# bjo5029/causal-vae

Hardware: AMD Instinct MI355X
Metric: training samples/sec on 128^3 vessel volumes (3D CausalVAE train step) (higher is better)
Workload: dtype bf16; 1 GPU; 3D vessel CausalVAE train step, 128^3 bf16 volumes (z-scored N(0,1)), batch 4/GPU, Adam lr 0.0001, ELBO = MSE-sum + 2000*MSE-sum(m) + KLD; global_batch=4, per_gpu_batch=4, parallelism=dp1, params=15346957

## Files before the change

### causal_vae_amd/_lib.py

```python
import ctypes as C
import os

import torch

_HERE = os.path.dirname(os.path.abspath(__file__))
LIB_PATH = os.environ.get("CVAE_HIP_LIB") or os.path.join(_HERE, "libcvae_hip.so")

F32, BF16, FP8 = 0, 1, 2
ACT_NONE, ACT_RELU, ACT_SIGMOID, ACT_LEAKY02, ACT_LEAKY001 = 0, 1, 2, 3, 4
_ACT = {None: ACT_NONE, "none": ACT_NONE, "relu": ACT_RELU, "sigmoid": ACT_SIGMOID, "leaky02": ACT_LEAKY02, "leaky001": ACT_LEAKY001}


class CvaeError(RuntimeError):
    pass


if not os.path.exists(LIB_PATH):
    raise ImportError(
        f"{LIB_PATH} is missing: build it with `python -c 'import __graft_entry__ as g; g.build()'` "
        "(or `make -C causal_vae_amd/csrc`).  causal_vae_amd has no CPU / eager fallback.")
lib = C.CDLL(LIB_PATH)

_p, _i64, _i, _f, _sz, _u64 = C.c_void_p, C.c_int64, C.c_int, C.c_float, C.c_size_t, C.c_uint64

SIGNATURES = {
    "cvae_version": [],
    "cvae_strerror": [_i],
    "cvae_ncs_to_nsc": [_p, _p, _i64, _i64, _i64, _i, _i, _p],
    "cvae_nsc_to_ncs": [_p, _p, _i64, _i64, _i64, _i, _i, _p],
    "cvae_cast": [_p, _p, _i64, _i, _i, _p],
    "cvae_copy_panels": [_p, _p, _p, _i, _p, _i64, _i64, _i64, _i, _p],
    "cvae_onehot_panel": [_p, _p, _i64, _i64, _i64, _i64, _p],
    "cvae_conv_pack_weight": [_p, _p, _i64, _i64, _i, _i, _i, _p],
    "cvae_conv_pack_weight_pairs": [_p, _p, _p, _p, _p, _p, _p, _p, _p, _i, _i, _i, _p],
    "cvae_conv_data_workspace_bytes": [_i64] * 9 + [_i, _i],
    "cvae_conv_down": [_p] * 7 + [_i64] * 9 + [_i, _i, _i, _p, _sz, _i, _p],
    "cvae_conv_up": [_p] * 7 + [_i64] * 9 + [_i, _i, _i, _p, _sz, _i, _i, _i64, _p],
    "cvae_conv_down_bwd_data": [_p] * 4 + [_i64] * 7 + [_i, _i, _i, _p, _sz, _i, _i, _p],
    "cvae_quantize_fp8": [_p, _i, _p, _i64, _f, _p, _p, _p],
    "cvae_conv_pack_weight_fp8": [_p, _p, _i64, _i64, _i, _i, _f, _p],
    "cvae_conv_up_c1_fp8in": [_p, _p, _p, _p, _f, _i64, _i64, _i64, _i64, _i64, _i, _i, _p],
    "cvae_absmax": [_p, _i, _i64, _p, _p],
    "cvae_conv_pack_weights_fp8": [_p, _p, _p, _p, _p, _p, _p, _i, _i, _p],
    "cvae_conv_fp8": [_i, _p, _p, _p, _p, _i, _p, _p, _f, _f, _p] + [_i64] * 9 + [_i, _i, _p, _sz, _i, _p, _p],
    "cvae_fp8_scale_update": [_p, _p, _p, _i, _f, _p, _p, _p, _i, _p, _p, _p],
    "cvae_conv_down_image_f8": [_p, _i, _p, _p, _p, _p, _p, _p, _p] + [_i64] * 8 + [_i, _i, _p],
    "cvae_conv_image_supported": [_p, _i64, _i, _i],
    "cvae_conv_down_image": [_p, _i, _p, _p, _p, _p] + [_i64] * 8 + [_i, _i, _i, _p],
    "cvae_conv_wgrad_image": [_p, _p, _i, _p, _p, _p, _sz] + [_i64] * 8 + [_i, _i, _p],
    "cvae_conv_wgrad_workspace_bytes": [_i64, _i64, _i],
    "cvae_conv_wgrad": [_p, _p, _p, _p, _i, _p, _sz] + [_i64] * 9 + [_i, _i, _p],
    "cvae_conv_wgrad_multi": [_i, _p, _p, _p, _p, _p, _p, _p, _p, _i, _i, _p],
    "cvae_channel_sum_workspace_bytes": [_i64, _i64, _i],
    "cvae_channel_sum": [_p, _p, _i64, _i64, _i, _p, _sz, _p],
    "cvae_act_fwd": [_p, _p, _i64, _i, _i, _p],
    "cvae_act_bwd": [_p, _p, _p, _i64, _i, _i, _p],
    "cvae_adaptive_avgpool_fwd": [_p, _p] + [_i64] * 9 + [_i, _p],
    "cvae_adaptive_avgpool_bwd": [_p, _p, _p] + [_i64] * 9 + [_i, _p],
    "cvae_upsample_linear_fwd": [_p, _p] + [_i64] * 8 + [_i, _p],
    "cvae_upsample_linear_bwd": [_p, _p] + [_i64] * 8 + [_i, _p],
    "cvae_linear_workspace_bytes": [_i64, _i64, _i64, _i],
    "cvae_linear_fwd": [_p, _p, _p, _p, _i64, _i64, _i64, _i64, _i64, _i, _i, _p, _sz, _p],
    "cvae_linear_bwd_data": [_p, _p, _p, _i64, _i64, _i64, _i64, _i64, _p, _i, _p, _i64, _i, _i, _p, _sz, _p],
    "cvae_linear_bwd_weight": [_p, _p, _p, _p, _i64, _i64, _i64, _i64, _i64, _p, _i, _i, _p, _sz, _p],
    "cvae_small_dense_supported": [_i64, _i64, _i64],
    "cvae_small_dense_workspace_bytes": [_i64, _i64, _i64],
    "cvae_small_dense_fwd": [_p, _p, _p, _p, _i64, _i64, _i64, _i64, _i64, _i, _p],
    "cvae_small_dense_bwd_data": [_p, _p, _p, _p, _i, _p, _i, _i64, _i64, _i64, _i64, _i64, _i64, _i64, _p],
    "cvae_small_dense_bwd_weight": [_p, _p, _p, _p, _p, _i, _i64, _i64, _i64, _i64, _i64, _i64, _p, _sz, _p],
    "cvae_bn1d_train_fwd": [_p] * 8 + [_i64, _i64, _f, _f, _p],
    "cvae_bn1d_train_bwd": [_p] * 8 + [_i64, _i64, _p],
    "cvae_bn1d_eval_fwd": [_p] * 6 + [_i64, _i64, _f, _p],
    "cvae_bn1d_stats": [_p, _p, _f, _p, _i64, _i64, _p],
    "cvae_bn1d_apply_stats": [_p] * 5 + [_f] + [_p] * 5 + [_i64, _i64, _f, _f, _p],
    "cvae_bn1d_bwd_sums": [_p] * 5 + [_i64, _i64, _p],
    "cvae_bn1d_bwd_apply": [_p] * 6 + [_f, _p, _i64, _i64, _p],
    "cvae_philox_normal": [_p, _i64, _u64, _u64, _u64, _p, _p],
    "cvae_philox_normal_advance": [_p, _i64, _u64, _u64, _u64, _p, _p],
    "cvae_reduce_workspace_bytes": [],
    "cvae_reparam_kld_fwd": [_p, _p, _p, _p, _p, _i64, _p, _sz, _p],
    "cvae_reparam_kld_bwd": [_p, _p, _f] + [_p] * 5 + [_i64, _p],
    "cvae_latent_head_fwd": [_p, _p, _p, _p, _p, _p, _i64, _i64, _p],
    "cvae_latent_head_bwd": [_p, _p, _p, _p, _p, _p, _p, _i64, _i64, _p],
    "cvae_sse_fwd": [_p, _p, _p, _i64, _p, _sz, _p],
    "cvae_sse_bwd": [_p, _p, _p, _f, _p, _i64, _p],
    "cvae_combine3": [_p, _f, _f, _p],
    "cvae_bce_fwd": [_p, _p, _p, _i64, _p, _sz, _p],
    "cvae_bce_bwd": [_p, _p, _p, _p, _i64, _p],
    "cvae_sum_fwd": [_p, _p, _i64, _p, _sz, _p],
    "cvae_wmse_sparsity_fwd": [_p, _p, _p, _p, _i64, _i64, _p, _sz, _p],
    "cvae_wmse_sparsity_bwd": [_p] * 6 + [_i64, _i64, _p],
    "cvae_gauss_nll_fwd": [_p, _p, _p, _p, _i64, _p, _sz, _p],
    "cvae_gauss_nll_bwd": [_p] * 6 + [_i64, _p],
    "cvae_softmax_ce_fwd": [_p, _p, _p, _i64, _i64, _p, _sz, _p],
    "cvae_softmax_ce_bwd": [_p, _p, _p, _p, _i64, _i64, _p],
    "cvae_uniform_kl_fwd": [_p, _p, _i64, _i64, _p, _sz, _p],
    "cvae_uniform_kl_bwd": [_p, _p, _p, _i64, _i64, _p],
    "cvae_adam_step": [_p, _p, _p, _p, _i64, _f, _f, _f, _f, _f, _f, _p, _p],
    "cvae_adam_multi": [_p, _p, _p, _p, _p, _i, _f, _f, _f, _f, _f, _f, _p, _p, _p],
    "cvae_multi_copy": [_p, _p, _p, _i, _p],
    "cvae_counter_add": [_p, _i, _p],
    "cvae_sqnorm": [_p, _p, _i64, _p, _sz, _p],
    "cvae_sqnorm_multi": [_p, _p, _i, _p, _p, _sz, _p],
    "cvae_weighted_sum": [_p, _p, _i, _p, _p, _i, _p],
    "cvae_scale": [_p, _i64, _p, _p],
    "cvae_clip_coef": [_p, _p, _f, _p],
    "cvae_up2x_supported": [_i64] * 7,
    "cvae_up2x_fwd": [_p, _p] + [_i64] * 7 + [_i, _p],
    "cvae_elbo_up2x_partials": [_i64] * 4,
    "cvae_elbo_up2x_fwd": [_p] * 6 + [_f, _p, _p, _p, _p, _p] + [_i64] * 9 + [_i, _p],
    "cvae_elbo_up2x_bwd": [_p] * 5 + [_f] + [_p] * 5 + [_i64] * 9 + [_i, _p],
    "cvae_conv3_to_k4": [_p, _p, _i64, _i64, _p],
    "cvae_k4_to_conv3_grad": [_p, _p, _i64, _i64, _p],
    "cvae_clamp_fwd": [_p, _p, _f, _f, _i64, _p],
    "cvae_clamp_bwd": [_p, _p, _p, _f, _f, _i64, _p],
    "cvae_bn2d_workspace_bytes": [_i64, _i64],
    "cvae_bn2d_fwd": [_p] * 8 + [_i64, _i64, _f, _f, _i, _i, _i, _p, _sz, _p],
    "cvae_bn2d_bwd": [_p] * 9 + [_i64, _i64, _i, _i, _p, _sz, _p],
    "cvae_fold_bn_conv": [_i] + [_p] * 11 + [_p],
    "cvae_fold_bn_conv_bwd": [_i] + [_p] * 14 + [_p],
    "cvae_vit_tokens": [_p, _i, _p, _p, _p, _i64, _i64, _p],
    "cvae_layernorm256": [_p, _i64, _p, _p, _p, _i64, _f, _i, _p],
    "cvae_token_gemm": [_p, _i64, _p, _p, _p, _i64, _p, _i64, _i64, _i64, _i64, _i, _i, _p],
    "cvae_mhsa_fwd": [_p] * 4 + [_i64] * 9 + [_i, _p],
    "cvae_mhsa_fwd_train": [_p] * 5 + [_i64] * 9 + [_i, _p],
    "cvae_mhsa_bwd_workspace_bytes": [_i64, _i64],
    "cvae_mhsa_bwd": [_p] * 9 + [_i64] * 15 + [_i, _p, _sz, _p],
    "cvae_token_gemm_gelu_train": [_p, _i64, _p, _p, _p, _i64, _p, _i64, _i64, _i64, _i64, _i, _p],
    "cvae_token_gemm_bwd_data": [_p, _i64, _i, _p, _p, _i64, _p, _i64, _p, _i64, _i, _i64, _i64, _i64, _i, _p],
    "cvae_token_gemm_wgrad_workspace_bytes": [_i64] * 3,
    "cvae_token_gemm_wgrad": [_p, _i64, _i, _p, _i64, _p, _p, _i64, _i64, _i64, _i, _p, _sz, _p],
    "cvae_layernorm256_bwd_workspace_bytes": [_i64],
    "cvae_layernorm256_bwd": [_p, _i64, _i, _p, _i64, _p, _p, _i64, _i, _p, _p, _i64, _f, _p, _sz, _p],
    "cvae_vit_tokens_bwd": [_p, _p, _p, _p, _i, _p, _i, _i64, _i64, _p],
    "cvae_conv_s1_weight_elems": [_i64, _i64, _i],
    "cvae_conv_s1_pack_weights": [_i, _p, _p, _p, _p],
    "cvae_conv_s1": [_p] * 5 + [_i64] * 5 + [_i, _i, _i, _p],
    "cvae_conv_s1_c1": [_p] * 4 + [_i64] * 4 + [_i, _i, _p],
    "cvae_latent_to_grid": [_p] * 4 + [_i64] * 4 + [_i, _p],
    "cvae_conv_s1_bwd_data": [_p] * 5 + [_i64] * 4 + [_i, _i, _i, _p],
    "cvae_conv_s1_c1_bwd_data": [_p] * 4 + [_i64] * 4 + [_i, _i, _p],
    "cvae_latent_to_grid_bwd_workspace_bytes": [_i64] * 4,
    "cvae_latent_to_grid_bwd": [_p] * 3 + [_i64] * 4 + [_i, _p, _sz, _p],
    "cvae_conv_s1_wgrad_workspace_bytes": [_i64] * 4 + [_i],
    "cvae_conv_s1_wgrad": [_p] * 4 + [_i64] * 4 + [_i, _i, _p, _sz, _p],
    "cvae_conv_s1_c1_wgrad_workspace_bytes": [_i64] * 3,
    "cvae_conv_s1_c1_wgrad": [_p] * 4 + [_i64] * 4 + [_i, _p, _sz, _p],
    "cvae_latent_to_grid_wgrad": [_p] * 4 + [_i64] * 4 + [_i, _p],
    "cvae_mlp_heads_fwd": [_p, _i, _p, _i, _i64, _p, _p, _p, _i64, _p, _i64, _p, _i64, _p, _i64, _i64, _p],
    "cvae_mlp_heads_train_workspace_bytes": [_p, _i, _p, _i, _i64],
    "cvae_mlp_heads_bwd_workspace_bytes": [_p, _i, _p, _i, _i64],
    "cvae_mlp_heads_train_fwd": [_p, _i, _p, _i, _p, _i64, _p, _p, _p, _i64, _p, _i64, _p, _i64, _p, _i64, _i64, _p, _sz, _p],
    "cvae_mlp_heads_bwd": [_p, _i, _p, _p, _p, _i, _p, _i64, _p, _p, _p, _i64, _p, _i64, _p, _i64, _p, _i64, _i64, _p, _sz, _p, _sz, _p],
    "cvae_row_diff_norms_workspace_bytes": [_i64, _i64, _i],
    "cvae_row_diff_norms": [_p] * 5 + [_i64, _i64, _i64, _i, _p, _sz, _p],
    "cvae_stack_mean_std": [_p, _i, _p, _p, _i64, _p],
    "cvae_bottleneck_sizes": [_p, _p, _p, _p, _p, _p],
    "cvae_bottleneck_fwd": [_p] * 10 + [_f, _f, _i, _p, _p, _p, _p, _p, _i, _p, _i, _p, _p],
    "cvae_bottleneck_bwd": [_p] * 12 + [_i, _p, _p, _p, _p, _i, _p, _p, _p],
    "cvae_bottleneck_bn_local_stats": [_p] * 5 + [_i64, _i64, _i64, _p],
    "cvae_bottleneck_bn_bwd_finish": [_p] * 7 + [_i, _p],
}
_RESTYPE = {"cvae_strerror": C.c_char_p, "cvae_conv_wgrad_workspace_bytes": _sz,
            "cvae_conv_data_workspace_bytes": _sz, "cvae_elbo_up2x_partials": _i64, "cvae_channel_sum_workspace_bytes": _sz,
            "cvae_linear_workspace_bytes": _sz, "cvae_reduce_workspace_bytes": _sz, "cvae_bn2d_workspace_bytes": _sz,
            "cvae_small_dense_workspace_bytes": _sz, "cvae_row_diff_norms_workspace_bytes": _sz,
            "cvae_mlp_heads_train_workspace_bytes": _sz, "cvae_mlp_heads_bwd_workspace_bytes": _sz,
            "cvae_conv_s1_weight_elems": _i64, "cvae_latent_to_grid_bwd_workspace_bytes": _sz,
            "cvae_conv_s1_wgrad_workspace_bytes": _sz, "cvae_conv_s1_c1_wgrad_workspace_bytes": _sz, "cvae_mhsa_bwd_workspace_bytes": _sz,
            "cvae_token_gemm_wgrad_workspace_bytes": _sz, "cvae_layernorm256_bwd_workspace_bytes": _sz}

for _name, _args in SIGNATURES.items():
    _fn = getattr(lib, _name)
    _fn.argtypes = _args
    _fn.restype = _RESTYPE.get(_name, _i)


class BottleneckDims(C.Structure):
    _fields_ = [(n, _i64) for n in ("M", "D", "H", "W", "C", "OD", "OH", "OW", "m_dim", "t_dim", "N1", "N2", "Z", "HM")]


BOTTLENECK_PARAMS = ("W1", "b1", "W2", "b2", "Wmu", "bmu", "Wlv", "blv", "Wm0", "bm0", "gamma", "beta", "Wm3", "bm3", "Wm5", "bm5", "Wd", "bd")
BOTTLENECK_SAVED = ("h1", "h2", "mu", "logvar", "xhat", "invstd", "a1n", "a2", "m_hat", "zm")


class BottleneckPtrs18(C.Structure):
    _fields_ = [(n, _p) for n in BOTTLENECK_PARAMS]


class BottleneckSaved(C.Structure):
    _fields_ = [(n, _p) for n in BOTTLENECK_SAVED]


class BottleneckNoise(C.Structure):
    _fields_ = [("seed", _u64), ("subsequence", _u64), ("call_counter", _p)]


HEADS_MAX_PANELS, HEADS_MAX_LAYERS, HEADS_MAX_WIDTH = 3, 3, 512


class HeadsPanel(C.Structure):
    _fields_ = [("ptr", _p), ("width", _i64), ("stride", _i64)]


class HeadsLayer(C.Structure):
    _fields_ = [("W", _p), ("b", _p), ("W2", _p), ("b2", _p), ("out", _i64), ("out_first", _i64), ("bn_weight", _p), ("bn_bias", _p), ("bn_mean", _p),
                ("bn_var", _p), ("bn_eps", _f), ("leaky", _i), ("slope", _f)]


class HeadsBnTrain(C.Structure):
    _fields_ = [("running_mean", _p), ("running_var", _p), ("num_batches_tracked", _p), ("momentum", _f)]


class HeadsLayerGrad(C.Structure):
    _fields_ = [(n, _p) for n in ("dW", "db", "dW2", "db2", "dgamma", "dbeta")]


class KernelTimer:

    def __init__(self):
        self.events = {}

    def run(self, name, fn, *args):
        s = torch.cuda.Event(enable_timing=True)
        e = torch.cuda.Event(enable_timing=True)
        s.record()
        rc = fn(*args)
        e.record()
        self.events.setdefault(name, []).append((s, e))
        return rc

    def summary(self):
        return {k: (len(v), sum(a.elapsed_time(b) for a, b in v) / len(v)) for k, v in self.events.items()}


TIMER = None


def timed(name, fn, *args):
    if TIMER is None:
        return fn(*args)
    return TIMER.run(name, fn, *args)


def strerror(code):
    return lib.cvae_strerror(code).decode()


def check(rc, what):
    if rc != 0:
        raise CvaeError(f"{what} failed: {strerror(rc)} (code {rc})")

# ... 27 lines not shown
```

### causal_vae_amd/csrc/bottleneck.hip

```cpp
#include "common.h"

#define BN_MAXM 16

namespace {

CVAE_TUNABLE(BN_NT, 0);
CVAE_TUNABLE(BN_FWD_UNROLL, 2);
CVAE_TUNABLE(BN_BWD_UNROLL, 8);
CVAE_TUNABLE(BN_FWD_SLICE, 4096);
CVAE_TUNABLE(BN_BWD_ROWS, 16);

struct TailDims { int M, N1, N2, Z, T, HM, DM, KS, P, NZ; };
struct TailParams {
    const float *b1, *W2, *b2, *Wmu, *bmu, *Wlv, *blv, *Wm0, *bm0, *gamma, *beta, *Wm3, *bm3, *Wm5, *bm5;
};
struct TailGrads {
    float *db1, *dW2, *db2, *dWmu, *dbmu, *dWlv, *dblv, *dWm0, *dbm0, *dgamma, *dbeta, *dWm3, *dbm3, *dWm5, *dbm5;
};
struct TailSaved { float *h1, *h2, *mu, *logvar, *xhat, *invstd, *a1n, *a2, *m_hat, *zm; };
struct MechFwdArgs { const float* t_onehot; float *running_mean, *running_var; long long* num_batches_tracked; float momentum, bn_eps; int bn_training;
                     const float* sync_stats; int sync_ranks; };
struct MechBwdArgs { const float *dzm_part, *g_mhat, *t_onehot; float *sync_dy, *sync_local; };
struct __attribute__((packed, aligned(4))) F4U { float x, y, z, w; };
typedef float v4f_u __attribute__((ext_vector_type(4), aligned(4)));
// ... 630 lines not shown
    __syncthreads();
    wg_linear_bwd(p.Wm0, gr.dWm0, gr.dbm0, dy, ts, nullptr, M, d.T, HM);
}

__global__ __launch_bounds__(256) void mulv_bwd_kernel(TailDims d, TailParams p, TailGrads gr, TailSaved sv, const float* __restrict__ dzm_part,
                                                       const float* __restrict__ g_mu, const float* __restrict__ g_logvar, const float* __restrict__ eps,
                                                       float* __restrict__ dh2) {
    extern __shared__ float lds[];
    const int M = d.M, tid = threadIdx.x, Z = d.Z, K4 = d.Z + d.DM;
    float* dzs = lds;
    float* dmu = dzs + M * K4;
    float* dlv = dmu + M * Z;
    float* h2c = dlv + M * Z;
    float* red = h2c + M * 16;
    const int k0 = blockIdx.x * 16;
    const int kl = tid & 15, q = tid >> 4, k = k0 + kl, kk = min(k, d.N2 - 1);
    constexpr int U = 4;
    float wm0[U], wl0[U];
#pragma unroll
    for (int u = 0; u < U; ++u) {
        const int nn = min(q + 16 * u, Z - 1);
        wm0[u] = p.Wmu[(size_t)nn * d.N2 + kk]; wl0[u] = p.Wlv[(size_t)nn * d.N2 + kk];
    }
    const int ie = min(tid, M * Z - 1);
    const float e_eps = eps[ie], e_lv = sv.logvar[ie], e_gm = g_mu ? g_mu[ie] : 0.f, e_gl = g_logvar ? g_logvar[ie] : 0.f;
    load_dzm(dzm_part, dzs, M * K4, d.NZ, lds_align16(red + 16 * M * 16));
    for (int i = tid; i < M * 16; i += 256) h2c[i] = (k0 + (i & 15) < d.N2) ? sv.h2[(i >> 4) * d.N2 + k0 + (i & 15)] : 0.f;
    __syncthreads();
    for (int i = tid; i < M * Z; i += 256) {
        const int m = i / Z, j = i - m * Z;
        const float dz = dzs[m * K4 + j];
        const bool first = i < 256;
        const float ve = first ? e_eps : eps[i], vl = first ? e_lv : sv.logvar[i];
        const float vgm = first ? e_gm : (g_mu ? g_mu[i] : 0.f), vgl = first ? e_gl : (g_logvar ? g_logvar[i] : 0.f);
        dmu[i] = dz + vgm;
        dlv[i] = dz * ve * 0.5f * __expf(0.5f * vl) + vgl;
    }
    __syncthreads();
    float acc[BN_MAXM];
#pragma unroll
    for (int m = 0; m < BN_MAXM; ++m) acc[m] = 0.f;
    if (k < d.N2) {
        for (int n0 = q; n0 < Z; n0 += 16 * U) {
            float wm[U], wl[U];
#pragma unroll
            for (int u = 0; u < U; ++u) {
                if (n0 == q) { wm[u] = wm0[u]; wl[u] = wl0[u]; }
                else {
                    const int nn = min(n0 + 16 * u, Z - 1);
                    wm[u] = p.Wmu[(size_t)nn * d.N2 + k]; wl[u] = p.Wlv[(size_t)nn * d.N2 + k];
                }
            }
#pragma unroll
            for (int u = 0; u < U; ++u) {
                const int n = n0 + 16 * u;
                if (n < Z) {
                    float gm = 0.f, gl = 0.f;
#pragma unroll
                    for (int m = 0; m < BN_MAXM; ++m)
                        if (m < M) {
                            acc[m] += dmu[m * Z + n] * wm[u] + dlv[m * Z + n] * wl[u];
                            gm += dmu[m * Z + n] * h2c[m * 16 + kl];
                            gl += dlv[m * Z + n] * h2c[m * 16 + kl];
                        }
                    gr.dWmu[(size_t)n * d.N2 + k] = gm;
                    gr.dWlv[(size_t)n * d.N2 + k] = gl;
                }
            }
        }
    }
#pragma unroll
    for (int m = 0; m < BN_MAXM; ++m)
        if (m < M) red[(q * M + m) * 16 + kl] = acc[m];
    __syncthreads();
    for (int i = tid; i < M * 16; i += 256) {
        const int m = i >> 4, c = i & 15;
        if (k0 + c < d.N2) {
            float v = 0.f;
#pragma unroll
            for (int qq = 0; qq < 16; ++qq) v += red[(qq * M + m) * 16 + c];
            dh2[m * d.N2 + k0 + c] = h2c[i] > 0.f ? v : 0.f;
        }
    }
    if (blockIdx.x == 0)
        for (int n = tid; n < Z; n += 256) {
            float bm = 0.f, bl = 0.f;
            for (int m = 0; m < M; ++m) { bm += dmu[m * Z + n]; bl += dlv[m * Z + n]; }
            gr.dbmu[n] = bm; gr.dblv[n] = bl;
        }
}

__global__ __launch_bounds__(256) void fc2_bwd_kernel(TailDims d, TailParams p, TailGrads gr, TailSaved sv, const float* __restrict__ dh2, float* __restrict__ g1) {
    extern __shared__ float lds[];
    const int M = d.M, tid = threadIdx.x, N = d.N2, K = d.N1;
    float* dhs = lds;
    float* h1c = dhs + M * N;
    float* red = h1c + M * 16;
    const int k0 = blockIdx.x * 16;
    const int kl = tid & 15, q = tid >> 4, k = k0 + kl;
    constexpr int U = 8;
    float w0[U];
#pragma unroll
    for (int u = 0; u < U; ++u) w0[u] = p.W2[(size_t)min(q + 16 * u, N - 1) * K + min(k, K - 1)];
    copy_g2l<4>(dhs, dh2, M * N);
    for (int i = tid; i < M * 16; i += 256) h1c[i] = (k0 + (i & 15) < K) ? sv.h1[(i >> 4) * K + k0 + (i & 15)] : 0.f;
    __syncthreads();
    float acc[BN_MAXM];
#pragma unroll
    for (int m = 0; m < BN_MAXM; ++m) acc[m] = 0.f;
    if (k < K) {
        for (int n0 = q; n0 < N; n0 += 16 * U) {
            float wv[U];
#pragma unroll
            for (int u = 0; u < U; ++u) wv[u] = (n0 == q) ? w0[u] : p.W2[(size_t)min(n0 + 16 * u, N - 1) * K + k];
#pragma unroll
            for (int u = 0; u < U; ++u) {
                const int n = n0 + 16 * u;
                if (n < N) {
                    float dw = 0.f;
#pragma unroll
                    for (int m = 0; m < BN_MAXM; ++m)
                        if (m < M) { acc[m] += dhs[m * N + n] * wv[u]; dw += dhs[m * N + n] * h1c[m * 16 + kl]; }
                    gr.dW2[(size_t)n * K + k] = dw;
                }
            }
        }
    }
#pragma unroll
    for (int m = 0; m < BN_MAXM; ++m)
        if (m < M) red[(q * M + m) * 16 + kl] = acc[m];
    __syncthreads();
    if (tid < 16 && k0 + tid < K) {
        float bsum = 0.f;
        for (int m = 0; m < M; ++m) {
            float v = 0.f;
            for (int qq = 0; qq < 16; ++qq) v += red[(qq * M + m) * 16 + tid];
            v = h1c[m * 16 + tid] > 0.f ? v : 0.f;
            g1[m * K + k0 + tid] = v;
            bsum += v;
        }
        gr.db1[k0 + tid] = bsum;
    }
    if (blockIdx.x == 0)
        for (int n = tid; n < N; n += 256) {
            float b = 0.f;
            for (int m = 0; m < M; ++m) b += dhs[m * N + n];
            gr.db2[n] = b;
        }
}

struct __attribute__((packed, aligned(4))) F2U { float x, y; };
template <int MT> struct SkinnyBwdCols { static constexpr int value = 4; using vec = F4U; };
template <> struct SkinnyBwdCols<16> { static constexpr int value = 2; using vec = F2U; };
template <int MT>
__global__ __launch_bounds__(256) void skinny_bwd_colwise_kernel(const float* __restrict__ g, const float* __restrict__ x, const float* __restrict__ Wt,
                                                                 float* __restrict__ dW, float* __restrict__ dxp, int M, int K, int N, int nslice, int F, int S,
                                                                 int NS, TailDims d, TailParams tp, TailGrads tg, TailSaved sv, MechBwdArgs mb) {
    extern __shared__ float dyn_lds[];
    if ((int)blockIdx.y == NS) {
        if (blockIdx.x == 0) mech_bwd(d, tp, tg, sv, mb.dzm_part, mb.g_mhat, mb.t_onehot, dyn_lds, mb.sync_dy, mb.sync_local);
        return;
    }
    __shared__ float gs[MT][64];
    constexpr int CPT = SkinnyBwdCols<MT>::value;
    const int k0 = (blockIdx.x * 256 + threadIdx.x) * CPT, ns = blockIdx.y;
    const int n0 = ns * nslice, n1 = min(N, n0 + nslice);
    const int nk = min(CPT, K - k0);
    float xv[MT][CPT], acc[MT][CPT];
#pragma unroll
    for (int m = 0; m < MT; ++m)
#pragma unroll
        for (int c = 0; c < CPT; ++c) { xv[m][c] = (m < M && c < nk) ? x[(size_t)m * K + k0 + c] : 0.f; acc[m][c] = 0.f; }
    for (int nb = n0; nb < n1; nb += 64) {
        const int cnt = min(64, n1 - nb);
        __syncthreads();
        for (int i = threadIdx.x; i < MT * 64; i += 256) {
            const int m = i >> 6, j = i & 63;
            gs[m][j] = (m < M && j < cnt) ? g[(size_t)m * N + nb + j] : 0.f;
        }
        __syncthreads();
        if (nk == CPT) {
            constexpr int UNR = MT >= 16 ? 2 : BN_BWD_UNROLL;
#pragma unroll UNR
            for (int j = 0; j < cnt; ++j) {
                typename SkinnyBwdCols<MT>::vec w = ld_stream<typename SkinnyBwdCols<MT>::vec>(Wt + (size_t)(nb + j) * K + k0), dw;
                const float* wf = (const float*)&w;
                float* dwf = (float*)&dw;
#pragma unroll
                for (int c = 0; c < CPT; ++c) dwf[c] = 0.f;
#pragma unroll
                for (int m = 0; m < MT; ++m) {
                    const float gv = gs[m][j];
#pragma unroll
                    for (int c = 0; c < CPT; ++c) { dwf[c] += gv * xv[m][c]; acc[m][c] += gv * wf[c]; }
                }
                st_stream<typename SkinnyBwdCols<MT>::vec>(dW + (size_t)(nb + j) * K + k0, dw);
            }
        } else if (nk > 0) {
            for (int j = 0; j < cnt; ++j)
                for (int c = 0; c < nk; ++c) {
                    const float w = Wt[(size_t)(nb + j) * K + k0 + c];
                    float dw = 0.f;
#pragma unroll
                    for (int m = 0; m < MT; ++m) { dw += gs[m][j] * xv[m][c]; acc[m][c] += gs[m][j] * w; }
                    dW[(size_t)(nb + j) * K + k0 + c] = dw;
                }
        }
    }
#pragma unroll
    for (int c = 0; c < CPT; ++c) {
        const int k = k0 + c;
        if (k < F) {
            const int ch = k / S, sp = k - ch * S, C = F / S;
#pragma unroll
            for (int m = 0; m < MT; ++m)
                if (m < M) dxp[(((size_t)ns * M + m) * S + sp) * C + ch] = acc[m][c];
        }
    }
}

template <typename T>
__global__ __launch_bounds__(256) void pool_bwd_kernel(const float* __restrict__ dxp, const T* __restrict__ y, T* __restrict__ dy, int NS, int M,
                                                       int D, int H, int W, int C, int OD, int OH, int OW, int relu_mask) {
    const int S = OD * OH * OW, b = blockIdx.y, s = blockIdx.x;
    const int ow = s % OW, oh = (s / OW) % OH, od = s / (OW * OH);
    const int d0 = pool_lo(od, D, OD), d1 = pool_hi(od, D, OD), h0 = pool_lo(oh, H, OH), h1 = pool_hi(oh, H, OH), w0 = pool_lo(ow, W, OW), w1 = pool_hi(ow, W, OW);
    const int nh = h1 - h0, nw = w1 - w0, nvox = (d1 - d0) * nh * nw;
    const float inv = 1.f / (float)nvox;
    __shared__ float4 part[4][64];
    __shared__ __attribute__((aligned(16))) float val[256];
    constexpr int EPP = 16 / sizeof(T);
    const int l = threadIdx.x & 63, q = threadIdx.x >> 6;
    for (int c0 = 0; c0 < C; c0 += 256) {
        const int cw = min(256, C - c0);
        float4 a = make_float4(0.f, 0.f, 0.f, 0.f);
        if (4 * l < cw) {
            constexpr int U = 8;
            for (int n0 = q; n0 < NS; n0 += 4 * U) {
                float4 v[U];
#pragma unroll
                for (int u = 0; u < U; ++u) v[u] = *(const float4*)(dxp + (((size_t)min(n0 + 4 * u, NS - 1) * M + b) * S + s) * C + c0 + 4 * l);
#pragma unroll
                for (int u = 0; u < U; ++u)
                    if (n0 + 4 * u < NS) { a.x += v[u].x; a.y += v[u].y; a.z += v[u].z; a.w += v[u].w; }
            }
        }
        part[q][l] = a;
        __syncthreads();
        if (q == 0) {
            const float4 b1 = part[1][l], b2 = part[2][l], b3 = part[3][l];
            *(float4*)(val + 4 * l) = make_float4((a.x + b1.x + b2.x + b3.x) * inv, (a.y + b1.y + b2.y + b3.y) * inv, (a.z + b1.z + b2.z + b3.z) * inv,
                                                  (a.w + b1.w + b2.w + b3.w) * inv);
        }
        __syncthreads();
        const int ppv = cw / EPP;
        for (int i = threadIdx.x; i < nvox * ppv; i += 256) {
            const int v = i / ppv, pc = (i - v * ppv) * EPP;
            const int ww = w0 + v % nw, hh = h0 + (v / nw) % nh, dd = d0 + v / (nw * nh);
            const size_t idx = ((((size_t)b * D + dd) * H + hh) * W + ww) * C + c0 + pc;
            union { uint4 u; T e[EPP]; } mk, o;
            if (relu_mask) mk.u = *(const uint4*)(y + idx);
#pragma unroll
            for (int e = 0; e < EPP; ++e) o.e[e] = from_f32<T>((!relu_mask || to_f32(mk.e[e]) > 0.f) ? val[pc + e] : 0.f);
            *(uint4*)(dy + idx) = o.u;
        }
        __syncthreads();
    }
}

size_t mech_fwd_lds(const TailDims& d) { return sizeof(float) * (size_t)d.M * (d.T + 2 * d.HM); }
size_t mech_bwd_lds(const TailDims& d) { return sizeof(float) * ((size_t)d.M * (d.Z + d.DM + d.DM + 5 * d.HM + d.T) + 4 * 256 + 4); }
size_t fc2_fwd_lds(const TailDims& d) { return sizeof(float) * (size_t)d.M * d.N1; }
size_t mulv_fwd_lds(const TailDims& d) { return sizeof(float) * (size_t)d.M * d.N2; }
size_t mulv_bwd_lds(const TailDims& d) { return sizeof(float) * ((size_t)d.M * (d.Z + d.DM) + 2 * (size_t)d.M * d.Z + 17 * (size_t)d.M * 16 + 4 * 256 + 4); }
size_t fc2_bwd_lds(const TailDims& d) { return sizeof(float) * ((size_t)d.M * d.N2 + 17 * (size_t)d.M * 16); }
size_t bn_finish_lds(const TailDims& d) { return sizeof(float) * (size_t)d.M * (d.HM + d.T); }
size_t dec_input_fwd_lds(int M, int K4) { return sizeof(float) * ((size_t)64 * (K4 | 1) + (size_t)M * K4 + (size_t)4 * M * 64); }
size_t dec_input_bwd_lds(int M, int K4) { return sizeof(float) * ((size_t)64 * (K4 | 1) + (size_t)M * K4 + (size_t)M * 64); }
template <typename F> auto with_mt(int M, F&& f) { return M <= 4 ? f(Int<4>{}) : (M <= 8 ? f(Int<8>{}) : f(Int<16>{})); }
int mt_of(int M) { return with_mt(M, [](auto mt) { return (int)decltype(mt)::value; }); }

constexpr size_t fwd_partial_static(int MT) { return sizeof(float) * 4 * 4 * MT; }
constexpr size_t bwd_colwise_static(int MT) { return sizeof(float) * 64 * MT; }
int fwd_lds_ready(const TailDims& d) {
    int rc = with_mt(d.M, [&](auto mt) {
        constexpr int MT = decltype(mt)::value;
        return cvae_allow_lds<skinny_fwd_partial_kernel<MT>>(mech_fwd_lds(d), fwd_partial_static(MT));
    });
    if (rc == CVAE_OK) rc = cvae_allow_lds<fc2_fwd_kernel>(fc2_fwd_lds(d));
    if (rc == CVAE_OK) rc = cvae_allow_lds<mulv_fwd_kernel>(mulv_fwd_lds(d));
    return rc;
}
int bwd_lds_ready(const TailDims& d) {
    const int rc = with_mt(d.M, [&](auto mt) {
        constexpr int MT = decltype(mt)::value;
        return cvae_allow_lds<skinny_bwd_colwise_kernel<MT>>(mech_bwd_lds(d), bwd_colwise_static(MT));
    });
    return rc == CVAE_OK ? cvae_allow_lds<fc2_bwd_kernel>(fc2_bwd_lds(d)) : rc;
}
TailParams tail_params(const cvae_bottleneck_params* w) {
    return TailParams{w->b1, w->W2, w->b2, w->Wmu, w->bmu, w->Wlv, w->blv, w->Wm0, w->bm0, w->gamma, w->beta, w->Wm3, w->bm3, w->Wm5, w->bm5};
}
TailGrads tail_grads(const cvae_bottleneck_grads* gr) {
    return TailGrads{gr->db1, gr->dW2, gr->db2, gr->dWmu, gr->dbmu, gr->dWlv, gr->dblv, gr->dWm0, gr->dbm0, gr->dgamma, gr->dbeta, gr->dWm3, gr->dbm3, gr->dWm5, gr->dbm5};
}
TailSaved tail_saved(const cvae_bottleneck_saved* sv) { return TailSaved{sv->h1, sv->h2, sv->mu, sv->logvar, sv->xhat, sv->invstd, sv->a1n, sv->a2, sv->m_hat, sv->zm}; }

}

static TailDims tail_dims(const cvae_bottleneck_dims* q, int KS, int P);
static bool dims_ok(const cvae_bottleneck_dims* q) {
    if (!q) return false;
    if (q->M < 1 || q->M > BN_MAXM) return false;
    if (q->C < 64 || q->C % 64 || q->D < 1 || q->H < 1 || q->W < 1 || q->OD < 1 || q->OH < 1 || q->OW < 1) return false;
    if (q->D % q->OD || q->H % q->OH || q->W % q->OW) return false;
    if (q->m_dim < 1 || q->t_dim < 1 || q->N1 < 4 || q->N2 < 1 || q->Z < 1 || q->HM < 1 || q->HM > 1024) return false;
    if (q->Z + q->m_dim > 128 || q->N1 > 4096 || q->N2 > 2048 || q->t_dim > 65536) return false;
    const TailDims d = tail_dims(q, 0, 0);
    const int MT = mt_of(d.M), K4 = d.Z + d.DM;
    const size_t need[] = {mech_fwd_lds(d) + fwd_partial_static(MT), fc2_fwd_lds(d), mulv_fwd_lds(d), dec_input_fwd_lds(d.M, K4), dec_input_bwd_lds(d.M, K4),
                           mulv_bwd_lds(d), fc2_bwd_lds(d), mech_bwd_lds(d) + bwd_colwise_static(MT), bn_finish_lds(d)};
    for (size_t b : need)
        if (b > CVAE_LDS_MAX) return false;
    return true;
}
static TailDims tail_dims(const cvae_bottleneck_dims* q, int KS, int P) {
    return TailDims{(int)q->M, (int)q->N1, (int)q->N2, (int)q->Z, (int)q->t_dim, (int)q->HM, (int)q->m_dim, KS, P, (int)(q->C * q->OD * q->OH * q->OW / 64)};
}
static int fwd_ksplit(int64_t K1) { int ks = (int)(K1 / BN_FWD_SLICE); return ks < 1 ? 1 : (ks > 8 ? 8 : ks); }
static int bwd_nsplit(int64_t N1) { int ns = (int)(N1 / BN_BWD_ROWS); return ns < 1 ? 1 : (ns > 64 ? 64 : ns); }

extern "C" int cvae_bottleneck_sizes(const cvae_bottleneck_dims* q, int64_t* K1, int64_t* K4, int64_t* fwd_partial_floats, int64_t* dzm_partial_floats,
                                     int64_t* dx_partial_floats) {
    if (!dims_ok(q)) return CVAE_E_BADSHAPE;
    const int64_t S = q->OD * q->OH * q->OW, F = q->C * S, k1 = F + q->m_dim + q->t_dim, k4 = q->Z + q->m_dim;
    if (K1) *K1 = k1;
    if (K4) *K4 = k4;
    if (fwd_partial_floats) *fwd_partial_floats = (int64_t)fwd_ksplit(k1) * q->M * q->N1;
    if (dzm_partial_floats) *dzm_partial_floats = (F / 64) * q->M * k4;
    if (dx_partial_floats) *dx_partial_floats = (int64_t)bwd_nsplit(q->N1) * q->M * F;
    return CVAE_OK;
}

extern "C" int cvae_bottleneck_bn_local_stats(const float* Wm0, const float* bm0, const float* t_onehot, const int64_t* t_labels, float* local_stats, int64_t M, int64_t t_dim,
                                              int64_t HM, void* stream) {
    if (M < 1 || M > BN_MAXM || t_dim < 1 || HM < 1 || HM > 1024) return CVAE_E_BADSHAPE;
    if (!Wm0 || !bm0 || !local_stats || (!t_onehot && !t_labels)) return CVAE_E_NULLPTR;
    hipLaunchKernelGGL(mech_bn_local_stats_kernel, dim3(1), dim3(256), 0, (hipStream_t)stream, Wm0, bm0, t_onehot, (const long long*)t_labels, local_stats, (int)M, (int)t_dim, (int)HM);
    CVAE_CHECK_LAUNCH();
    return CVAE_OK;
}

extern "C" int cvae_bottleneck_fwd(const cvae_bottleneck_dims* q, const cvae_bottleneck_params* w, const void* y_cl, const float* m, float* t_onehot,
                                   const int64_t* t_labels, float* eps, float* running_mean, float* running_var, long long* num_batches_tracked, float momentum,
                                   float bn_eps, int bn_training, float* xcat, float* partial, float* dzm_acc, const cvae_bottleneck_saved* sv, void* dec_cl, int dtype,
                                   const float* bn_rank_stats, int bn_ranks, const cvae_bottleneck_noise* noise, void* stream) {
    if (!dims_ok(q)) return CVAE_E_BADSHAPE;
    if (noise && !noise->call_counter) return CVAE_E_NULLPTR;
    const NoiseDraw nz = noise ? NoiseDraw{eps, (int)(q->M * q->Z), noise->seed, noise->subsequence, noise->call_counter} : NoiseDraw{nullptr, 0, 0, 0, nullptr};
    if (bn_rank_stats && (bn_ranks < 1 || !bn_training)) return CVAE_E_BADSHAPE;
    if (dtype != CVAE_F32 && dtype != CVAE_BF16) return CVAE_E_DTYPE;
    if (!w || !sv || !y_cl || !m || !t_onehot || !eps || !xcat || !partial || !dec_cl) return CVAE_E_NULLPTR;
    if (bn_training && q->M * (bn_rank_stats ? bn_ranks : 1) < 2) return CVAE_E_BADSHAPE;
    if (!bn_training && (!running_mean || !running_var)) return CVAE_E_NULLPTR;
    if (fwd_lds_ready(tail_dims(q, 0, 0)) != CVAE_OK) return CVAE_E_LAUNCH;
    hipStream_t st = (hipStream_t)stream;
    const int M = (int)q->M, S = (int)(q->OD * q->OH * q->OW), C = (int)q->C, F = C * S;
    const int K1 = F + (int)q->m_dim + (int)q->t_dim, K4 = (int)(q->Z + q->m_dim), KS = fwd_ksplit(K1);
    with_dtype(dtype, [&](auto tv) {
        using T = decltype(tv);
        hipLaunchKernelGGL(pool_cat_fwd_kernel<T>, dim3(S + 1, M), dim3(256), 0, st, (const T*)y_cl, m, t_onehot, (const long long*)t_labels, xcat, (int)q->D, (int)q->H, (int)q->W, C,
                           (int)q->OD, (int)q->OH, (int)q->OW, (int)q->m_dim, (int)q->t_dim, K1, nz);
    });
    CVAE_CHECK_LAUNCH();
    const TailDims d = tail_dims(q, KS, 0);
    const TailParams p = tail_params(w);
    const TailSaved s = tail_saved(sv);
    const MechFwdArgs ma{t_onehot, running_mean, running_var, num_batches_tracked, momentum, bn_eps, bn_training, bn_rank_stats, bn_ranks};
    with_mt(M, [&](auto mt) {
        hipLaunchKernelGGL(skinny_fwd_partial_kernel<decltype(mt)::value>, dim3((unsigned)((q->N1 + 3) / 4), (unsigned)(KS + 1)), dim3(256), mech_fwd_lds(d), st,
                           (const float*)xcat, w->W1, partial, M, K1, (int)q->N1, (K1 + KS - 1) / KS, KS, d, p, s, ma);
    });
    CVAE_CHECK_LAUNCH();
    hipLaunchKernelGGL(fc2_fwd_kernel, dim3((unsigned)((q->N2 + 3) / 4)), dim3(256), fc2_fwd_lds(d), st, d, p, s, (const float*)partial);
    CVAE_CHECK_LAUNCH();
    hipLaunchKernelGGL(mulv_fwd_kernel, dim3((unsigned)((q->Z + 3) / 4)), dim3(256), mulv_fwd_lds(d), st, d, p, s, eps);
    CVAE_CHECK_LAUNCH();
    const size_t lds_d = dec_input_fwd_lds(M, K4);
    with_dtype(dtype, [&](auto tv) {
        using T = decltype(tv);
        hipLaunchKernelGGL(dec_input_fwd_kernel<T>, dim3(C * S / 64), dim3(256), lds_d, st, (const float*)sv->zm, w->Wd, w->bd, (T*)dec_cl, M, K4, S, C);
    });
    CVAE_CHECK_LAUNCH();
    return CVAE_OK;
}

extern "C" int cvae_bottleneck_bn_bwd_finish(const cvae_bottleneck_dims* q, const cvae_bottleneck_params* w, const cvae_bottleneck_grads* gr, const cvae_bottleneck_saved* sv,
                                             const float* t_onehot, const float* bn_dy, const float* bn_sums, int bn_ranks, void* stream) {
    if (!dims_ok(q) || bn_ranks < 1) return CVAE_E_BADSHAPE;
    if (!w || !gr || !sv || !t_onehot || !bn_dy || !bn_sums) return CVAE_E_NULLPTR;
    const TailDims d = tail_dims(q, 0, 0);
    const TailParams p = tail_params(w);
    const TailGrads g = tail_grads(gr);
    const TailSaved s = tail_saved(sv);
    if (cvae_allow_lds<mech_bn_finish_kernel>(bn_finish_lds(d)) != CVAE_OK) return CVAE_E_LAUNCH;
    hipLaunchKernelGGL(mech_bn_finish_kernel, dim3(1), dim3(256), bn_finish_lds(d), (hipStream_t)stream, d, p, g, s, t_onehot, bn_dy, bn_sums,
                       bn_ranks);
    CVAE_CHECK_LAUNCH();
    return CVAE_OK;
}

extern "C" int cvae_bottleneck_bwd(const cvae_bottleneck_dims* q, const cvae_bottleneck_params* w, const cvae_bottleneck_grads* gr, const cvae_bottleneck_saved* sv,
                                   const void* g_dec_cl, const float* g_mu, const float* g_logvar, const float* g_mhat, const float* t_onehot, const float* eps,
                                   const float* xcat, const void* y_cl, int relu_mask, float* dzm_partial, float* g1, float* dx_partial, void* dy_cl, int dtype,
                                   float* bn_dy, float* bn_local_sums, void* stream) {
    if (!dims_ok(q)) return CVAE_E_BADSHAPE;
    if ((bn_dy == nullptr) != (bn_local_sums == nullptr)) return CVAE_E_NULLPTR;
    if (dtype != CVAE_F32 && dtype != CVAE_BF16) return CVAE_E_DTYPE;
    if (!w || !gr || !sv || !g_dec_cl || !t_onehot || !eps || !xcat || !y_cl || !dzm_partial || !g1 || !dx_partial || !dy_cl) return CVAE_E_NULLPTR;
    if (bwd_lds_ready(tail_dims(q, 0, 0)) != CVAE_OK) return CVAE_E_LAUNCH;
    hipStream_t st = (hipStream_t)stream;
    const int M = (int)q->M, S = (int)(q->OD * q->OH * q->OW), C = (int)q->C, F = C * S;
    const int K1 = F + (int)q->m_dim + (int)q->t_dim, K4 = (int)(q->Z + q->m_dim), NS = bwd_nsplit(q->N1), P = S;
    const size_t lds_d = dec_input_bwd_lds(M, K4);
    with_dtype(dtype, [&](auto tv) {
        using T = decltype(tv);
        hipLaunchKernelGGL(dec_input_bwd_kernel<T>, dim3(F / 64), dim3(256), lds_d, st, (const T*)g_dec_cl, (const float*)sv->zm, w->Wd, gr->dWd, gr->dbd, dzm_partial, M, K4, S, C);
    });
    CVAE_CHECK_LAUNCH();
    const TailDims d = tail_dims(q, 0, P);
    const TailParams p = tail_params(w);
    const TailGrads g = tail_grads(gr);
    const TailSaved s = tail_saved(sv);
    float* dh2 = g1 + (size_t)M * q->N1;
    hipLaunchKernelGGL(mulv_bwd_kernel, dim3((unsigned)((q->N2 + 15) / 16)), dim3(256), mulv_bwd_lds(d), st,
                       d, p, g, s, (const float*)dzm_partial, g_mu, g_logvar, eps, dh2);
    CVAE_CHECK_LAUNCH();
    hipLaunchKernelGGL(fc2_bwd_kernel, dim3((unsigned)((q->N1 + 15) / 16)), dim3(256), fc2_bwd_lds(d), st, d, p, g, s,
                       (const float*)dh2, g1);
    CVAE_CHECK_LAUNCH();
    const MechBwdArgs mb{dzm_partial, g_mhat, t_onehot, bn_dy, bn_local_sums};
    with_mt(M, [&](auto mt) {
        constexpr int MT = decltype(mt)::value, COLS = 256 * SkinnyBwdCols<MT>::value;
        hipLaunchKernelGGL(skinny_bwd_colwise_kernel<MT>, dim3((unsigned)((K1 + COLS - 1) / COLS), (unsigned)(NS + 1)), dim3(256), mech_bwd_lds(d), st, (const float*)g1, xcat,
                           w->W1, gr->dW1, dx_partial, M, K1, (int)q->N1, ((int)q->N1 + NS - 1) / NS, F, S, NS, d, p, g, s, mb);
    });
    CVAE_CHECK_LAUNCH();
    with_dtype(dtype, [&](auto tv) {
        using T = decltype(tv);
        hipLaunchKernelGGL(pool_bwd_kernel<T>, dim3(S, M), dim3(256), 0, st, (const float*)dx_partial, (const T*)y_cl, (T*)dy_cl, NS, M, (int)q->D, (int)q->H, (int)q->W, C,
                           (int)q->OD, (int)q->OH, (int)q->OW, relu_mask);
    });
    CVAE_CHECK_LAUNCH();
    return CVAE_OK;
}
```

### causal_vae_amd/csrc/common.h

```cpp
#pragma once
#include <hip/hip_runtime.h>
#include <stdint.h>
#include <type_traits>
#include "../../include/cvae_hip.h"

typedef __bf16 bf16;
typedef __attribute__((ext_vector_type(8))) __bf16 bf16x8;
typedef __attribute__((ext_vector_type(4))) __bf16 bf16x4;
typedef __attribute__((ext_vector_type(16))) float f32x16;
typedef __attribute__((ext_vector_type(4))) float f32x4;

#define CVAE_WAVE 64

#define CVAE_CHECK_LAUNCH()                                   \
    do {                                                      \
        hipError_t e__ = hipGetLastError();                   \
        if (e__ != hipSuccess) return CVAE_E_LAUNCH;          \
    } while (0)

constexpr size_t CVAE_LDS_MAX = 160 * 1024, CVAE_LDS_OPT_IN = 48 * 1024;
template <auto KERN> int cvae_allow_lds(size_t dynamic_bytes, size_t static_bytes = 0) {
    if (dynamic_bytes <= CVAE_LDS_OPT_IN) return CVAE_OK;
    const int limit = (int)(CVAE_LDS_MAX - static_bytes);
    return hipFuncSetAttribute((const void*)KERN, hipFuncAttributeMaxDynamicSharedMemorySize, limit) == hipSuccess ? CVAE_OK : CVAE_E_LAUNCH;
// ... 16 lines not shown
static inline int cvae_grid_1d(int64_t n, int block, int max_blocks = 256 * 8) {
    int64_t g = (n + block - 1) / block;
    if (g < 1) g = 1;
    if (g > max_blocks) g = max_blocks;
    return (int)g;
}

struct fp8 { unsigned char b; };
#define CVAE_FP8_MAX 448.f

__device__ __forceinline__ float to_f32(float x) { return x; }
__device__ __forceinline__ float to_f32(bf16 x) { return (float)x; }
__device__ __forceinline__ float to_f32(fp8 x) { return __builtin_amdgcn_cvt_f32_fp8((int)x.b, 0); }
template <typename T> __device__ __forceinline__ T from_f32(float x);
template <> __device__ __forceinline__ float from_f32<float>(float x) { return x; }
template <> __device__ __forceinline__ bf16 from_f32<bf16>(float x) { return (bf16)x; }
typedef __bf16 cvae_bf16x2 __attribute__((ext_vector_type(2)));
typedef float cvae_f32x2 __attribute__((ext_vector_type(2)));
__device__ __forceinline__ uint32_t pack2_bf16(float a, float b) {
    const cvae_f32x2 f = {a, b};
    const cvae_bf16x2 r = __builtin_convertvector(f, cvae_bf16x2);
    return __builtin_bit_cast(uint32_t, r);
}
template <> __device__ __forceinline__ fp8 from_f32<fp8>(float x) {
    x = fminf(fmaxf(x, -CVAE_FP8_MAX), CVAE_FP8_MAX);
    return fp8{(unsigned char)(__builtin_amdgcn_cvt_pk_fp8_f32(x, x, 0, false) & 0xff)};
}
template <int N> __device__ __forceinline__ void load_f32(const float* p, float (&v)[N]) {
#pragma unroll
    for (int q = 0; q < N / 4; ++q) {
        const float4 f = ((const float4*)p)[q];
        v[4 * q] = f.x; v[4 * q + 1] = f.y; v[4 * q + 2] = f.z; v[4 * q + 3] = f.w;
    }
}
template <int N> __device__ __forceinline__ void load_f32(const bf16* p, float (&v)[N]) {
    typedef bf16 vec __attribute__((ext_vector_type(N), aligned(N < 8 ? 8 : 16)));
    const vec q = *(const vec*)p;
#pragma unroll
    for (int i = 0; i < N; ++i) v[i] = (float)q[i];
}
template <int N> __device__ __forceinline__ void store_from_f32(float* p, const float (&v)[N]) {
#pragma unroll
    for (int q = 0; q < N / 4; ++q) ((float4*)p)[q] = make_float4(v[4 * q], v[4 * q + 1], v[4 * q + 2], v[4 * q + 3]);
}
template <int N> __device__ __forceinline__ void store_from_f32(bf16* p, const float (&v)[N]) {
    typedef uint32_t vec __attribute__((ext_vector_type(N / 2), aligned(N < 8 ? 8 : 16)));
    vec q;
#pragma unroll
    for (int i = 0; i < N / 2; ++i) q[i] = pack2_bf16(v[2 * i], v[2 * i + 1]);
    *(vec*)p = q;
}
inline bool aligned16(const void* p) { return ((uintptr_t)p & 15) == 0; }

__device__ __forceinline__ float wave_sum(float v) {
#pragma unroll
    for (int o = 32; o > 0; o >>= 1) v += __shfl_xor(v, o, 64);
    return v;
}
__device__ __forceinline__ float wave_max(float v) {
#pragma unroll
    for (int o = 32; o > 0; o >>= 1) v = fmaxf(v, __shfl_xor(v, o, 64));
    return v;
}
__device__ __forceinline__ float block_sum(float v, float* red) {
    v = wave_sum(v);
    const int lane = threadIdx.x & 63, wid = threadIdx.x >> 6, nw = (blockDim.x + 63) >> 6;
    __syncthreads();
    if (lane == 0) red[wid] = v;
    __syncthreads();
    float r = 0.f;
    if (threadIdx.x == 0)
        for (int i = 0; i < nw; ++i) r += red[i];
    return r;
}

__device__ __forceinline__ uint2 pack8_fp8(const float (&v)[8], float mul) {
    float c[8];
#pragma unroll
    for (int q = 0; q < 8; ++q) c[q] = __builtin_amdgcn_fmed3f(v[q] * mul, -CVAE_FP8_MAX, CVAE_FP8_MAX);
    int lo = __builtin_amdgcn_cvt_pk_fp8_f32(c[0], c[1], 0, false);
    lo = __builtin_amdgcn_cvt_pk_fp8_f32(c[2], c[3], lo, true);
    int hi = __builtin_amdgcn_cvt_pk_fp8_f32(c[4], c[5], 0, false);
    hi = __builtin_amdgcn_cvt_pk_fp8_f32(c[6], c[7], hi, true);
    return make_uint2((unsigned)lo, (unsigned)hi);
}
__device__ __forceinline__ uint4 fp8_pair_to_16(uint2 a, uint2 b) {
    const auto x = __builtin_amdgcn_permlane32_swap(a.x, b.x, false, false);
    const auto y = __builtin_amdgcn_permlane32_swap(a.y, b.y, false, false);
    return make_uint4(x[0], y[0], x[1], y[1]);
}
struct F8Side {
    const float* dscale;
    fp8* out8;
    unsigned* amax;
    const unsigned* mask_bits;
    unsigned* bits_out;
};
__device__ __forceinline__ unsigned mask_bytes_to_dword(unsigned b0, unsigned b1) {
    const unsigned a = b0 | (b1 << 16);
    const auto x = __builtin_amdgcn_permlane32_swap(a, a, false, false);
    return (x[0] & 0xffu) | ((x[1] & 0xffu) << 8) | (((x[0] >> 16) & 0xffu) << 16) | ((x[1] >> 16) << 24);
}
__device__ __forceinline__ unsigned mask_byte_of(const float (&v)[8]) {
    unsigned b = 0;
#pragma unroll
    for (int q = 0; q < 8; ++q) b |= (v[q] > 0.f ? 1u : 0u) << q;
    return b;
}
#define REGROUP_D32(acc, v)                                                                                                                      \
    _Pragma("unroll") for (int i_ = 0; i_ < 4; ++i_) {                                                                                           \
        const auto lo_ = __builtin_amdgcn_permlane32_swap(__float_as_uint((acc)[i_]), __float_as_uint((acc)[4 + i_]), false, false);              \
        const auto hi_ = __builtin_amdgcn_permlane32_swap(__float_as_uint((acc)[8 + i_]), __float_as_uint((acc)[12 + i_]), false, false);         \
        (v)[0][i_] = __uint_as_float(lo_[0]); (v)[0][4 + i_] = __uint_as_float(lo_[1]);                                                          \
        (v)[1][i_] = __uint_as_float(hi_[0]); (v)[1][4 + i_] = __uint_as_float(hi_[1]);                                                          \
    }
__device__ __forceinline__ void amax_publish_wg(unsigned* slots, float amx, unsigned wg, float* red) {
#pragma unroll
    for (int o = 32; o > 0; o >>= 1) amx = fmaxf(amx, __shfl_xor(amx, o, 64));
    const int nw = (blockDim.x + 63) >> 6;
    if ((threadIdx.x & 63) == 0) red[threadIdx.x >> 6] = amx;
    __syncthreads();
    if (threadIdx.x == 0) {
        float m = red[0];
        for (int i = 1; i < nw; ++i) m = fmaxf(m, red[i]);
        if (m > 0.f) atomicMax(slots + (wg & (CVAE_AMAX_SLOTS - 1)), __float_as_uint(m));
    }
}

__device__ __forceinline__ float apply_act(float v, int act) {
    switch (act) {
        case CVAE_ACT_RELU: return v > 0.f ? v : 0.f;
        case CVAE_ACT_SIGMOID: return 1.f / (1.f + __expf(-v));
        case CVAE_ACT_LEAKY02: return v > 0.f ? v : 0.2f * v;
        case CVAE_ACT_LEAKY001: return v > 0.f ? v : 0.01f * v;
        default: return v;
    }
}
__device__ __forceinline__ float relu_f32(float v) {
    float r;
    asm("v_max_f32_e32 %0, 0, %1" : "=v"(r) : "v"(v));
    return r;
}
template <int EPI> __device__ __forceinline__ float apply_act_t(float v, int act) {
    if (EPI == 0) return v;
    if (EPI == 1) return relu_f32(v);
    return apply_act(v, act);
}
#define CVAE_EPI_OF(act) ((act) == CVAE_ACT_NONE ? 0 : ((act) == CVAE_ACT_RELU ? 1 : 2))
template <int V> using Int = std::integral_constant<int, V>;
template <typename F> auto with_nd(int nd, F&& f) { return nd == 3 ? f(Int<3>{}) : f(Int<2>{}); }
template <typename F> auto with_dtype(int dtype, F&& f) { return dtype == CVAE_BF16 ? f(bf16{}) : f(float{}); }
template <typename F> auto with_epi(int act, F&& f) { return CVAE_EPI_OF(act) == 0 ? f(Int<0>{}) : (CVAE_EPI_OF(act) == 1 ? f(Int<1>{}) : f(Int<2>{})); }
template <typename F> auto with_bool(bool b, F&& f) { return b ? f(std::true_type{}) : f(std::false_type{}); }
__device__ __forceinline__ float act_grad_from_out(float y, int act) {
    switch (act) {
        case CVAE_ACT_RELU: return y > 0.f ? 1.f : 0.f;
        case CVAE_ACT_SIGMOID: return y * (1.f - y);
        case CVAE_ACT_LEAKY02: return y > 0.f ? 1.f : 0.2f;
        case CVAE_ACT_LEAKY001: return y > 0.f ? 1.f : 0.01f;
        default: return 1.f;
    }
}

__device__ __forceinline__ uint4 fp8x8_to_bf16x8(uint2 c) {
    const auto a = __builtin_amdgcn_cvt_pk_f32_fp8((int)c.x, false), b = __builtin_amdgcn_cvt_pk_f32_fp8((int)c.x, true);
    const auto d = __builtin_amdgcn_cvt_pk_f32_fp8((int)c.y, false), e = __builtin_amdgcn_cvt_pk_f32_fp8((int)c.y, true);
    return make_uint4(pack2_bf16(a[0], a[1]), pack2_bf16(b[0], b[1]), pack2_bf16(d[0], d[1]), pack2_bf16(e[0], e[1]));
}

__device__ __forceinline__ void philox_round(uint32_t& c0, uint32_t& c1, uint32_t& c2, uint32_t& c3, uint32_t k0, uint32_t k1) {
    const uint64_t p0 = (uint64_t)0xD2511F53u * c0, p1 = (uint64_t)0xCD9E8D57u * c2;
    const uint32_t n0 = (uint32_t)(p1 >> 32) ^ c1 ^ k0, n1 = (uint32_t)p1, n2 = (uint32_t)(p0 >> 32) ^ c3 ^ k1, n3 = (uint32_t)p0;
    c0 = n0; c1 = n1; c2 = n2; c3 = n3;
}
__device__ __forceinline__ void philox_normal4(uint64_t ctr, uint64_t subseq, uint64_t seed, float v[4]) {
    uint32_t c0 = (uint32_t)ctr, c1 = (uint32_t)(ctr >> 32), c2 = (uint32_t)subseq, c3 = (uint32_t)(subseq >> 32);
    uint32_t k0 = (uint32_t)seed, k1 = (uint32_t)(seed >> 32);
#pragma unroll
    for (int r = 0; r < 10; ++r) { philox_round(c0, c1, c2, c3, k0, k1); k0 += 0x9E3779B9u; k1 += 0xBB67AE85u; }
    const float u0 = ((float)(c0 >> 8) + 0.5f) * (1.f / 16777216.f), u1 = ((float)(c1 >> 8) + 0.5f) * (1.f / 16777216.f);
    const float u2 = ((float)(c2 >> 8) + 0.5f) * (1.f / 16777216.f), u3 = ((float)(c3 >> 8) + 0.5f) * (1.f / 16777216.f);
    const float r0 = sqrtf(-2.f * logf(u0)), r1 = sqrtf(-2.f * logf(u2));
    sincosf(6.283185307179586f * u1, &v[1], &v[0]);
    sincosf(6.283185307179586f * u3, &v[3], &v[2]);
    v[0] *= r0; v[1] *= r0; v[2] *= r1; v[3] *= r1;
}

template <typename I> __device__ __forceinline__ I pool_lo(I o, I in, I out) { return (o * in) / out; }
template <typename I> __device__ __forceinline__ I pool_hi(I o, I in, I out) { return ((o + 1) * in + out - 1) / out; }

template <typename I> struct LinTap { I i0, i1; float w0, w1; };
template <typename I> __device__ __forceinline__ LinTap<I> lin_tap(I o, I in, float scale) {
    float s = scale * ((float)o + 0.5f) - 0.5f;
    if (s < 0.f) s = 0.f;
    LinTap<I> t;
    t.i0 = (I)s;
    if (t.i0 > in - 1) t.i0 = in - 1;
    t.i1 = t.i0 + ((t.i0 < in - 1) ? 1 : 0);
    t.w1 = s - (float)t.i0;
    t.w0 = 1.f - t.w1;
    return t;
}
struct Win4 { int j0; float w[4]; };
template <typename I> __device__ __forceinline__ Win4 win4(int i, int in, int out, float scale, bool strided) {
    Win4 r;
    if (!strided) { r.j0 = i; r.w[0] = 1.f; r.w[1] = r.w[2] = r.w[3] = 0.f; return r; }
    r.j0 = 2 * i - 1;
#pragma unroll
    for (int c = 0; c < 4; ++c) {
        const int j = r.j0 + c;
        float wv = 0.f;
        if (j >= 0 && j < out) {
            const LinTap<I> t = lin_tap<I>(j, in, scale);
            wv = (t.i0 == i ? t.w0 : 0.f) + (t.i1 == i ? t.w1 : 0.f);
        }
        r.w[c] = wv;
    }
    return r;
}
```

### causal_vae_amd/csrc/losses.hip

```cpp
#include "common.h"

#define RED_BLOCK 256
#define RED_MAX_BLOCKS 1024
#define RED_MAX_OUT 2
extern "C" size_t cvae_reduce_workspace_bytes(void) { return (size_t)RED_MAX_BLOCKS * RED_MAX_OUT * sizeof(float); }
static inline int red_grid_ws(int64_t items, int block, int cap, int nout, const void* ws, size_t ws_bytes) {
    int g = cvae_grid_1d(items, block, cap < RED_MAX_BLOCKS ? cap : RED_MAX_BLOCKS);
    if (g > 1 && (!ws || ws_bytes < (size_t)g * nout * sizeof(float))) g = 1;
    return g;
}
__device__ __forceinline__ void red_emit(float s, float* __restrict__ out, float* __restrict__ ws, int o) {
    if (gridDim.x == 1) out[o] += s;
    else ws[(size_t)o * gridDim.x + blockIdx.x] = s;
}
template <int NOUT>
__global__ __launch_bounds__(RED_BLOCK) void red_finish_kernel(const float* __restrict__ ws, int nblocks, float* __restrict__ out) {
    __shared__ float red[RED_BLOCK / 64];
#pragma unroll
    for (int o = 0; o < NOUT; ++o) {
        float acc = 0.f;
        for (int i = threadIdx.x; i < nblocks; i += RED_BLOCK) acc += ws[(size_t)o * nblocks + i];
        const float s = block_sum(acc, red);
        if (threadIdx.x == 0) out[o] += s;
    }
// ... 425 lines not shown
    s1 = wave_sum(s1); s2 = wave_sum(s2);
    const float inv = 1.f / (float)B;
    for (int64_t i = lane; i < B; i += 64) {
        const float g = dy[i * F + f], xh = (x[i * F + f] - mean) * rstd;
        dx[i * F + f] = ww * rstd * (g - s1 * inv - xh * s2 * inv);
    }
    if (lane == 0) { if (dw) dw[f] = s2; if (db) db[f] = s1; }
}
extern "C" int cvae_bn1d_train_bwd(const float* dy, const float* x, const float* w, const float* save_mean, const float* save_rstd,
                                   float* dx, float* dw, float* db, int64_t B, int64_t F, void* stream) {
    if (B < 2 || F <= 0) return CVAE_E_BADSHAPE;
    if (!dy || !x || !save_mean || !save_rstd || !dx) return CVAE_E_NULLPTR;
    hipLaunchKernelGGL(bn1d_train_bwd_kernel, dim3((unsigned)((F * 64 + 255) / 256)), dim3(256), 0, (hipStream_t)stream, dy, x, w, save_mean, save_rstd, dx, dw, db, B, F);
    CVAE_CHECK_LAUNCH();
    return CVAE_OK;
}
__global__ void bn1d_stats_kernel(const float* __restrict__ x, const float* __restrict__ mean_sum, float inv_n, float* __restrict__ out, int64_t B, int64_t F) {
    const int lane = threadIdx.x & 63;
    const int64_t f = (blockIdx.x * (int64_t)blockDim.x + threadIdx.x) >> 6;
    if (f >= F) return;
    const float mean = mean_sum ? mean_sum[f] * inv_n : 0.f;
    float s = 0.f;
    for (int64_t i = lane; i < B; i += 64) { const float d = x[i * F + f] - mean; s += mean_sum ? d * d : d; }
    s = wave_sum(s);
    if (lane == 0) out[f] = s;
}
extern "C" int cvae_bn1d_stats(const float* x, const float* mean_sum, float inv_n, float* out, int64_t B, int64_t F, void* stream) {
    if (B < 1 || F <= 0) return CVAE_E_BADSHAPE;
    if (!x || !out) return CVAE_E_NULLPTR;
    hipLaunchKernelGGL(bn1d_stats_kernel, dim3((unsigned)((F * 64 + 255) / 256)), dim3(256), 0, (hipStream_t)stream, x, mean_sum, inv_n, out, B, F);
    CVAE_CHECK_LAUNCH();
    return CVAE_OK;
}
__global__ void bn1d_apply_stats_kernel(const float* __restrict__ x, const float* __restrict__ w, const float* __restrict__ b, const float* __restrict__ mean_sum,
                                        const float* __restrict__ sqdev_sum, float inv_n, float* __restrict__ y, float* __restrict__ save_mean,
                                        float* __restrict__ save_rstd, float* __restrict__ rmean, float* __restrict__ rvar, int64_t B, int64_t F, float momentum,
                                        float eps, int update_running) {
    const int lane = threadIdx.x & 63;
    const int64_t f = (blockIdx.x * (int64_t)blockDim.x + threadIdx.x) >> 6;
    if (f >= F) return;
    const float mean = mean_sum[f] * inv_n, var = sqdev_sum[f] * inv_n, rstd = rsqrtf(var + eps);
    const float ww = w ? w[f] : 1.f, bb = b ? b[f] : 0.f;
    for (int64_t i = lane; i < B; i += 64) y[i * F + f] = (x[i * F + f] - mean) * rstd * ww + bb;
    if (lane == 0) {
        save_mean[f] = mean;
        save_rstd[f] = rstd;
        if (update_running && rmean) rmean[f] = (1.f - momentum) * rmean[f] + momentum * mean;
        const float n = 1.f / inv_n;
        if (update_running && rvar) rvar[f] = (1.f - momentum) * rvar[f] + momentum * (sqdev_sum[f] / (n - 1.f));
    }
}
extern "C" int cvae_bn1d_apply_stats(const float* x, const float* w, const float* b, const float* mean_sum, const float* sqdev_sum, float inv_n, float* y,
                                     float* save_mean, float* save_rstd, float* running_mean, float* running_var, int64_t B, int64_t F, float momentum,
                                     float eps, void* stream) {
    if (B < 1 || F <= 0 || !(inv_n > 0.f) || inv_n > 0.5f) return CVAE_E_BADSHAPE;
    if (!x || !mean_sum || !sqdev_sum || !y || !save_mean || !save_rstd) return CVAE_E_NULLPTR;
    hipLaunchKernelGGL(bn1d_apply_stats_kernel, dim3((unsigned)((F * 64 + 255) / 256)), dim3(256), 0, (hipStream_t)stream, x, w, b, mean_sum, sqdev_sum, inv_n, y,
                       save_mean, save_rstd, running_mean, running_var, B, F, momentum, eps, 1);
    CVAE_CHECK_LAUNCH();
    return CVAE_OK;
}
__global__ void bn1d_bwd_sums_kernel(const float* __restrict__ dy, const float* __restrict__ x, const float* __restrict__ save_mean,
                                     const float* __restrict__ save_rstd, float* __restrict__ sums, int64_t B, int64_t F) {
    const int lane = threadIdx.x & 63;
    const int64_t f = (blockIdx.x * (int64_t)blockDim.x + threadIdx.x) >> 6;
    if (f >= F) return;
    const float mean = save_mean[f], rstd = save_rstd[f];
    float s1 = 0.f, s2 = 0.f;
    for (int64_t i = lane; i < B; i += 64) { const float g = dy[i * F + f]; s1 += g; s2 += g * (x[i * F + f] - mean) * rstd; }
    s1 = wave_sum(s1); s2 = wave_sum(s2);
    if (lane == 0) { sums[f] = s1; sums[F + f] = s2; }
}
extern "C" int cvae_bn1d_bwd_sums(const float* dy, const float* x, const float* save_mean, const float* save_rstd, float* sums, int64_t B, int64_t F, void* stream) {
    if (B < 1 || F <= 0) return CVAE_E_BADSHAPE;
    if (!dy || !x || !save_mean || !save_rstd || !sums) return CVAE_E_NULLPTR;
    hipLaunchKernelGGL(bn1d_bwd_sums_kernel, dim3((unsigned)((F * 64 + 255) / 256)), dim3(256), 0, (hipStream_t)stream, dy, x, save_mean, save_rstd, sums, B, F);
    CVAE_CHECK_LAUNCH();
    return CVAE_OK;
}
__global__ void bn1d_bwd_apply_kernel(const float* __restrict__ dy, const float* __restrict__ x, const float* __restrict__ w, const float* __restrict__ save_mean,
                                      const float* __restrict__ save_rstd, const float* __restrict__ sums, float inv_n, float* __restrict__ dx, int64_t B, int64_t F) {
    for (int64_t i = blockIdx.x * (int64_t)blockDim.x + threadIdx.x; i < B * F; i += (int64_t)gridDim.x * blockDim.x) {
        const int64_t f = i % F;
        const float rstd = save_rstd[f], xh = (x[i] - save_mean[f]) * rstd;
        dx[i] = (w ? w[f] : 1.f) * rstd * (dy[i] - sums[f] * inv_n - xh * sums[F + f] * inv_n);
    }
}
extern "C" int cvae_bn1d_bwd_apply(const float* dy, const float* x, const float* w, const float* save_mean, const float* save_rstd, const float* sums, float inv_n,
                                   float* dx, int64_t B, int64_t F, void* stream) {
    if (B < 1 || F <= 0 || !(inv_n > 0.f)) return CVAE_E_BADSHAPE;
    if (!dy || !x || !save_mean || !save_rstd || !sums || !dx) return CVAE_E_NULLPTR;
    hipLaunchKernelGGL(bn1d_bwd_apply_kernel, dim3(cvae_grid_1d(B * F, 256)), dim3(256), 0, (hipStream_t)stream, dy, x, w, save_mean, save_rstd, sums, inv_n, dx, B, F);
    CVAE_CHECK_LAUNCH();
    return CVAE_OK;
}
__global__ void bn1d_eval_fwd_kernel(const float* __restrict__ x, const float* __restrict__ w, const float* __restrict__ b, const float* __restrict__ rm,
                                     const float* __restrict__ rv, float* __restrict__ y, int64_t n, int64_t F, float eps) {
    for (int64_t i = blockIdx.x * (int64_t)blockDim.x + threadIdx.x; i < n; i += (int64_t)gridDim.x * blockDim.x) {
        const int64_t f = i % F;
        y[i] = (x[i] - rm[f]) / sqrtf(rv[f] + eps) * (w ? w[f] : 1.f) + (b ? b[f] : 0.f);
    }
}
extern "C" int cvae_bn1d_eval_fwd(const float* x, const float* w, const float* b, const float* rm, const float* rv, float* y, int64_t B, int64_t F, float eps, void* stream) {
    if (B < 0 || F <= 0) return CVAE_E_BADSHAPE;
    if (B == 0) return CVAE_OK;
    if (!x || !rm || !rv || !y) return CVAE_E_NULLPTR;
    hipLaunchKernelGGL(bn1d_eval_fwd_kernel, dim3(cvae_grid_1d(B * F, 256)), dim3(256), 0, (hipStream_t)stream, x, w, b, rm, rv, y, B * F, F, eps);
    CVAE_CHECK_LAUNCH();
    return CVAE_OK;
}

template <bool ADVANCE>
__global__ void philox_normal_kernel(float* __restrict__ out, int64_t n, uint64_t seed, uint64_t offset, uint64_t subseq, int* __restrict__ call_dev) {
    if (call_dev) offset += ((uint64_t)(unsigned)(*call_dev)) << 24;
    if (ADVANCE) {
        __syncthreads();
        if (threadIdx.x == 0) *call_dev += 1;
    }
    const int64_t n4 = (n + 3) >> 2;
    for (int64_t i = blockIdx.x * (int64_t)blockDim.x + threadIdx.x; i < n4; i += (int64_t)gridDim.x * blockDim.x) {
        float v[4];
        philox_normal4(offset + (uint64_t)i, subseq, seed, v);
        for (int j = 0; j < 4; ++j) if (i * 4 + j < n) out[i * 4 + j] = v[j];
    }
}
extern "C" int cvae_philox_normal(float* out, int64_t n, uint64_t seed, uint64_t offset, uint64_t subsequence, const int* call_counter, void* stream) {
    if (n < 0) return CVAE_E_BADSHAPE;
    if (n == 0) return CVAE_OK;
    if (!out) return CVAE_E_NULLPTR;
    hipLaunchKernelGGL(philox_normal_kernel<false>, dim3(cvae_grid_1d((n + 3) / 4, 256)), dim3(256), 0, (hipStream_t)stream, out, n, seed, offset, subsequence, (int*)call_counter);
    CVAE_CHECK_LAUNCH();
    return CVAE_OK;
}
__global__ void add_int_kernel(int* c, int delta);
extern "C" int cvae_philox_normal_advance(float* out, int64_t n, uint64_t seed, uint64_t offset, uint64_t subsequence, int* call_counter, void* stream) {
    if (n < 0) return CVAE_E_BADSHAPE;
    if (!call_counter) return CVAE_E_NULLPTR;
    if (n > 0 && !out) return CVAE_E_NULLPTR;
    if (n > 0 && n <= 16384) {
        hipLaunchKernelGGL(philox_normal_kernel<true>, dim3(1), dim3(256), 0, (hipStream_t)stream, out, n, seed, offset, subsequence, call_counter);
    } else {
        if (n > 0) hipLaunchKernelGGL(philox_normal_kernel<false>, dim3(cvae_grid_1d((n + 3) / 4, 256)), dim3(256), 0, (hipStream_t)stream, out, n, seed, offset, subsequence, call_counter);
        hipLaunchKernelGGL(add_int_kernel, dim3(1), dim3(64), 0, (hipStream_t)stream, call_counter, 1);
    }
    CVAE_CHECK_LAUNCH();
    return CVAE_OK;
}

__device__ __forceinline__ void adam1(float& p, float g, float& m, float& v, float b1, float b2, float eps, float step, float rbc2) {
    m = b1 * m + (1.f - b1) * g;
    v = b2 * v + (1.f - b2) * g * g;
    p -= step * (m / (sqrtf(v) * rbc2 + eps));
}
__global__ void adam_kernel(float* __restrict__ p, const float* __restrict__ g, float* __restrict__ m, float* __restrict__ v, int64_t n,
                            float lr, float b1, float b2, float eps, float bc1, float bc2, const float* __restrict__ gscale) {
    const float gs = gscale ? *gscale : 1.f;
    const float step = lr / bc1, rbc2 = 1.f / sqrtf(bc2);
    const int64_t n4 = n >> 2;
    const bool vec = ((((uintptr_t)p) | ((uintptr_t)g) | ((uintptr_t)m) | ((uintptr_t)v)) & 15) == 0;
    if (vec) {
        for (int64_t i = blockIdx.x * (int64_t)blockDim.x + threadIdx.x; i < n4; i += (int64_t)gridDim.x * blockDim.x) {
            float4 P = ((float4*)p)[i], G = ((const float4*)g)[i], M = ((float4*)m)[i], V = ((float4*)v)[i];
            adam1(P.x, G.x * gs, M.x, V.x, b1, b2, eps, step, rbc2);
            adam1(P.y, G.y * gs, M.y, V.y, b1, b2, eps, step, rbc2);
            adam1(P.z, G.z * gs, M.z, V.z, b1, b2, eps, step, rbc2);
            adam1(P.w, G.w * gs, M.w, V.w, b1, b2, eps, step, rbc2);
            ((float4*)p)[i] = P; ((float4*)m)[i] = M; ((float4*)v)[i] = V;
        }
        for (int64_t i = (n4 << 2) + blockIdx.x * (int64_t)blockDim.x + threadIdx.x; i < n; i += (int64_t)gridDim.x * blockDim.x)
            adam1(p[i], g[i] * gs, m[i], v[i], b1, b2, eps, step, rbc2);
    } else {
        for (int64_t i = blockIdx.x * (int64_t)blockDim.x + threadIdx.x; i < n; i += (int64_t)gridDim.x * blockDim.x)
            adam1(p[i], g[i] * gs, m[i], v[i], b1, b2, eps, step, rbc2);
    }
}
extern "C" int cvae_adam_step(float* p, const float* g, float* m, float* v, int64_t n, float lr, float b1, float b2, float eps,
                              float bc1, float bc2, const float* gscale, void* stream) {
    if (n < 0 || bc1 <= 0.f || bc2 <= 0.f) return CVAE_E_BADSHAPE;
    if (n == 0) return CVAE_OK;
    if (!p || !g || !m || !v) return CVAE_E_NULLPTR;
    hipLaunchKernelGGL(adam_kernel, dim3(cvae_grid_1d((n + 3) / 4, 256)), dim3(256), 0, (hipStream_t)stream, p, g, m, v, n, lr, b1, b2, eps, bc1, bc2, gscale);
    CVAE_CHECK_LAUNCH();
    return CVAE_OK;
}
#define ADAM_MAX_TENSORS 64
#define ADAM_SPAN 4096
#define ADAM_MULTI_SPAN 1024
struct AdamTable {
    float* p[ADAM_MAX_TENSORS];
    const float* g[ADAM_MAX_TENSORS];
    float* m[ADAM_MAX_TENSORS];
    float* v[ADAM_MAX_TENSORS];
    long long n[ADAM_MAX_TENSORS];
    int blk_start[ADAM_MAX_TENSORS + 1];
    int count;
};
template <int SPAN, bool NT = false>
__global__ __launch_bounds__(256) void adam_multi_kernel(AdamTable tb, float lr, float b1, float b2, float eps, float bc1, float bc2,
                                                         const int* __restrict__ step_dev, const float* __restrict__ gscale) {
    int ti = 0;
    while (ti + 1 < tb.count && (int)blockIdx.x >= tb.blk_start[ti + 1]) ++ti;
    if (step_dev) { const float st = (float)(*step_dev); bc1 = 1.f - powf(b1, st); bc2 = 1.f - powf(b2, st); }
    const float gs = gscale ? *gscale : 1.f;
    const float step = lr / bc1, rbc2 = 1.f / sqrtf(bc2);
    float* p = tb.p[ti]; const float* g = tb.g[ti]; float* m = tb.m[ti]; float* v = tb.v[ti];
    const long long n = tb.n[ti];
    const long long base = (long long)((int)blockIdx.x - tb.blk_start[ti]) * SPAN;
    const long long end = min(n, base + SPAN);
    const bool vec = ((((uintptr_t)p) | ((uintptr_t)g) | ((uintptr_t)m) | ((uintptr_t)v)) & 15) == 0;
    if (vec && end - base == SPAN) {
#pragma unroll
        for (int k = 0; k < SPAN / (256 * 4); ++k) {
            const long long i = base / 4 + k * 256 + threadIdx.x;
            float4 P, G, M, V;
            if (NT) {
                typedef float f4v __attribute__((ext_vector_type(4)));
                f4v a = __builtin_nontemporal_load((f4v*)p + i), b = __builtin_nontemporal_load((const f4v*)g + i);
                f4v c = __builtin_nontemporal_load((f4v*)m + i), d = __builtin_nontemporal_load((f4v*)v + i);
                P = make_float4(a.x, a.y, a.z, a.w); G = make_float4(b.x, b.y, b.z, b.w); M = make_float4(c.x, c.y, c.z, c.w); V = make_float4(d.x, d.y, d.z, d.w);
            } else { P = ((float4*)p)[i]; G = ((const float4*)g)[i]; M = ((float4*)m)[i]; V = ((float4*)v)[i]; }
            adam1(P.x, G.x * gs, M.x, V.x, b1, b2, eps, step, rbc2);
            adam1(P.y, G.y * gs, M.y, V.y, b1, b2, eps, step, rbc2);
            adam1(P.z, G.z * gs, M.z, V.z, b1, b2, eps, step, rbc2);
            adam1(P.w, G.w * gs, M.w, V.w, b1, b2, eps, step, rbc2);
            if (NT) {
                typedef float f4v __attribute__((ext_vector_type(4)));
                f4v a = {P.x, P.y, P.z, P.w}, c = {M.x, M.y, M.z, M.w}, d = {V.x, V.y, V.z, V.w};
                __builtin_nontemporal_store(a, (f4v*)p + i); __builtin_nontemporal_store(c, (f4v*)m + i); __builtin_nontemporal_store(d, (f4v*)v + i);
            }
            else { ((float4*)p)[i] = P; ((float4*)m)[i] = M; ((float4*)v)[i] = V; }
        }
    } else {
        for (long long i = base + threadIdx.x; i < end; i += 256) adam1(p[i], g[i] * gs, m[i], v[i], b1, b2, eps, step, rbc2);
    }
}
extern "C" int cvae_adam_multi(float* const* p, const float* const* g, float* const* m, float* const* v, const int64_t* n, int count,
                               float lr, float b1, float b2, float eps, float bc1, float bc2, const int* step_dev, const float* gscale, void* stream) {
    if (count < 0) return CVAE_E_BADSHAPE;
    if (count == 0) return CVAE_OK;
    if (!p || !g || !m || !v || !n) return CVAE_E_NULLPTR;
    if (!step_dev && (bc1 <= 0.f || bc2 <= 0.f)) return CVAE_E_BADSHAPE;
    const int span = ADAM_MULTI_SPAN;
    for (int c0 = 0; c0 < count; c0 += ADAM_MAX_TENSORS) {
        AdamTable tb;
        const int cnt = (count - c0 < ADAM_MAX_TENSORS) ? count - c0 : ADAM_MAX_TENSORS;
        int blocks = 0, used = 0;
        for (int i = 0; i < cnt; ++i) {
            const int64_t ni = n[c0 + i];
            if (ni < 0) return CVAE_E_BADSHAPE;
            if (ni == 0) continue;
            if (!p[c0 + i] || !g[c0 + i] || !m[c0 + i] || !v[c0 + i]) return CVAE_E_NULLPTR;
            tb.p[used] = p[c0 + i]; tb.g[used] = g[c0 + i]; tb.m[used] = m[c0 + i]; tb.v[used] = v[c0 + i]; tb.n[used] = ni;
            tb.blk_start[used] = blocks;
            blocks += (int)((ni + span - 1) / span);
            ++used;
        }
        if (!used) continue;
        tb.blk_start[used] = blocks;
        tb.count = used;
        hipLaunchKernelGGL((adam_multi_kernel<ADAM_MULTI_SPAN, true>), dim3(blocks), dim3(256), 0, (hipStream_t)stream, tb, lr, b1, b2, eps, bc1, bc2, step_dev, gscale);
        CVAE_CHECK_LAUNCH();
    }
    return CVAE_OK;
}
struct CopyTable {
    const float* src[ADAM_MAX_TENSORS];
    float* dst[ADAM_MAX_TENSORS];
    long long n[ADAM_MAX_TENSORS];
    int blk_start[ADAM_MAX_TENSORS + 1];
    int count;
};
__global__ __launch_bounds__(256) void multi_copy_kernel(CopyTable tb) {
    int ti = 0;
    while (ti + 1 < tb.count && (int)blockIdx.x >= tb.blk_start[ti + 1]) ++ti;
    const float* s = tb.src[ti];
    float* d = tb.dst[ti];
    const long long base = (long long)((int)blockIdx.x - tb.blk_start[ti]) * ADAM_SPAN, end = min(tb.n[ti], base + ADAM_SPAN);
    if (((((uintptr_t)s) | ((uintptr_t)d)) & 15) == 0 && end - base == ADAM_SPAN) {
#pragma unroll
        for (int k = 0; k < ADAM_SPAN / (256 * 4); ++k) ((float4*)d)[base / 4 + k * 256 + threadIdx.x] = ((const float4*)s)[base / 4 + k * 256 + threadIdx.x];
    } else {
        for (long long i = base + threadIdx.x; i < end; i += 256) d[i] = s[i];
    }
}
extern "C" int cvae_multi_copy(const float* const* src, float* const* dst, const int64_t* n, int count, void* stream) {
    if (count < 0) return CVAE_E_BADSHAPE;
    if (count == 0) return CVAE_OK;
    if (!src || !dst || !n) return CVAE_E_NULLPTR;
    for (int c0 = 0; c0 < count; c0 += ADAM_MAX_TENSORS) {
        CopyTable tb;
        const int cnt = (count - c0 < ADAM_MAX_TENSORS) ? count - c0 : ADAM_MAX_TENSORS;
        int blocks = 0, used = 0;
        for (int i = 0; i < cnt; ++i) {
            const int64_t ni = n[c0 + i];
            if (ni < 0) return CVAE_E_BADSHAPE;
            if (ni == 0) continue;
            if (!src[c0 + i] || !dst[c0 + i]) return CVAE_E_NULLPTR;
            tb.src[used] = src[c0 + i]; tb.dst[used] = dst[c0 + i]; tb.n[used] = ni; tb.blk_start[used] = blocks;
            blocks += (int)((ni + ADAM_SPAN - 1) / ADAM_SPAN);
            ++used;
        }
        if (!used) continue;
        tb.blk_start[used] = blocks;
        tb.count = used;
        hipLaunchKernelGGL(multi_copy_kernel, dim3(blocks), dim3(256), 0, (hipStream_t)stream, tb);
        CVAE_CHECK_LAUNCH();
    }
    return CVAE_OK;
}
__global__ void add_int_kernel(int* c, int delta) { if (threadIdx.x == 0 && blockIdx.x == 0) *c += delta; }
extern "C" int cvae_counter_add(int* counter, int delta, void* stream) {
    if (!counter) return CVAE_E_NULLPTR;
    hipLaunchKernelGGL(add_int_kernel, dim3(1), dim3(64), 0, (hipStream_t)stream, counter, delta);
    CVAE_CHECK_LAUNCH();
    return CVAE_OK;
}

__global__ void scale_kernel(float* __restrict__ g, int64_t n, const float* __restrict__ scale) {
    const float s = *scale;
    for (int64_t i = blockIdx.x * (int64_t)blockDim.x + threadIdx.x; i < n; i += (int64_t)gridDim.x * blockDim.x) g[i] *= s;
}
extern "C" int cvae_scale(float* g, int64_t n, const float* scale, void* stream) {
    if (n < 0) return CVAE_E_BADSHAPE;
    if (n == 0) return CVAE_OK;
    if (!g || !scale) return CVAE_E_NULLPTR;
    hipLaunchKernelGGL(scale_kernel, dim3(cvae_grid_1d(n, 256)), dim3(256), 0, (hipStream_t)stream, g, n, scale);
    CVAE_CHECK_LAUNCH();
    return CVAE_OK;
}
__global__ void clip_coef_kernel(const float* __restrict__ sq, float* __restrict__ scale, float max_norm) {
    if (threadIdx.x == 0 && blockIdx.x == 0) *scale = fminf(1.f, max_norm / (sqrtf(*sq) + 1e-6f));
}
struct Scalars8 { const float* t[8]; float w[8]; int n; };
__global__ void weighted_sum_kernel(Scalars8 a, const float* __restrict__ g, float* __restrict__ out, int backward) {
    if (threadIdx.x != 0 || blockIdx.x != 0) return;
    if (backward) {
        const float gv = g ? *g : 1.f;
        for (int i = 0; i < a.n; ++i) out[i] = a.w[i] * gv;
    } else {
        float s = 0.f;
        for (int i = 0; i < a.n; ++i) { const float v = a.w[i] * *a.t[i]; out[1 + i] = v; s += v; }
        out[0] = s;
    }
}
extern "C" int cvae_weighted_sum(const float* const* terms, const float* weights, int count, const float* g, float* out, int backward, void* stream) {
    if (count < 1 || count > 8) return CVAE_E_BADSHAPE;
    if (!weights || !out || (!backward && !terms)) return CVAE_E_NULLPTR;
    Scalars8 a;
    a.n = count;
    for (int i = 0; i < count; ++i) {
        a.t[i] = backward ? nullptr : terms[i];
        if (!backward && !terms[i]) return CVAE_E_NULLPTR;
        a.w[i] = weights[i];
    }
    hipLaunchKernelGGL(weighted_sum_kernel, dim3(1), dim3(64), 0, (hipStream_t)stream, a, g, out, backward);
    CVAE_CHECK_LAUNCH();
    return CVAE_OK;
}
extern "C" int cvae_clip_coef(const float* sq, float* scale, float max_norm, void* stream) {
    if (!sq || !scale) return CVAE_E_NULLPTR;
    hipLaunchKernelGGL(clip_coef_kernel, dim3(1), dim3(64), 0, (hipStream_t)stream, sq, scale, max_norm);
    CVAE_CHECK_LAUNCH();
    return CVAE_OK;
}
```

### causal_vae_amd/graph.py

```python
import torch

from . import ops

from ._lib import CvaeError
from .optim import FusedAdam


def _capture(graph, **kw):
    return torch.cuda.graph(graph, capture_error_mode="thread_local", **kw)


def _check_sync_bn_capturable(model):
    import torch.distributed as dist
    if not (dist.is_available() and dist.is_initialized()):
        return
    for mod in model.modules():
        if getattr(mod, "sync", False):
            group = getattr(mod, "sync_group", None)
            if dist.get_world_size(group) > 1 and dist.get_backend(group) != "nccl":
                raise CvaeError("GraphedTrainStep: SyncBatchNorm collectives can only be captured on an RCCL ('nccl') process group; run the eager train_step "
                                f"on '{dist.get_backend(group)}'")


class GraphedTrainStep:
    def __init__(self, model, optimizer, batch, loss_fn=None, reducer=None, warmup=3, overlap_exchange=False):
        if not isinstance(optimizer, FusedAdam) or not optimizer.device_step:
            raise CvaeError("GraphedTrainStep needs FusedAdam(..., device_step=True): the step count must live on the device")
        self.model, self.opt, self.reducer = model, optimizer, reducer
        _check_sync_bn_capturable(model)
        self.x, self.m, self.t = (b.clone() for b in batch)
        self.loss_fn = loss_fn
        side = torch.cuda.Stream()
        side.wait_stream(torch.cuda.current_stream())
        with torch.cuda.stream(side):
            for _ in range(warmup):
                self._fwd_bwd()
                self._reduce_eager()
                self.opt.step()
        torch.cuda.current_stream().wait_stream(side)
        torch.cuda.synchronize()
        self.g1 = torch.cuda.CUDAGraph()
        self.g2 = self.g1b = None
        if overlap_exchange:
            self._capture_split()
        elif reducer is None or not reducer.active():
            with _capture(self.g1):
                self.out = self._fwd_bwd()
                self.opt.step()
        else:
            with _capture(self.g1):
                self.out = self._fwd_bwd()
                reducer.pack()
            self.g2 = torch.cuda.CUDAGraph()
            with _capture(self.g2, pool=self.g1.pool()):
                reducer.unpack()
                self.opt.step()

    def _fwd_bwd(self):
        self.opt.zero_grad(set_to_none=True)
        if self.loss_fn is None:
            bump = self.opt.claim_step_counter(self.x.device) if not getattr(self.opt, "_early", None) else None
            res = self.model.forward_elbo(self.x, self.m, self.t, bump=bump)
        else:
            res = self.loss_fn(self.model(self.x, self.m, self.t), self.x, self.m)
        ops.backward_from(res[0])
        return tuple(r.detach() for r in res)

    def _capture_split(self):
        from .parallel import GradAllReducer
        if self.loss_fn is not None or not hasattr(self.model, "early_gradient_parameters"):
            raise CvaeError("overlap_exchange needs the model's own forward_elbo and early_gradient_parameters()")
        params_a = [p for p in self.model.early_gradient_parameters() if p.requires_grad]
        ids_a = {id(p) for p in params_a}
        params_b = [p for p in self.model.parameters() if p.requires_grad and id(p) not in ids_a]
        group = self.reducer.group if self.reducer is not None else None
        always = self.reducer.always_exchange if self.reducer is not None else False
        comm = self.reducer.comm if self.reducer is not None else None
        self.red_a, self.red_b = GradAllReducer(params_a, group, always, comm), GradAllReducer(params_b, group, always, comm)
        self.red_a.pack(); self.red_b.pack()
        torch.cuda.synchronize()
        if hasattr(torch.autograd.graph, "set_warn_on_accumulate_grad_stream_mismatch"):
            torch.autograd.graph.set_warn_on_accumulate_grad_stream_mismatch(False)
        cap = torch.cuda.Stream()
        with _capture(self.g1, stream=cap):
            self.opt.zero_grad(set_to_none=True)
            res = self.model.forward_elbo(self.x, self.m, self.t, bump=self.opt.claim_step_counter(self.x.device))
            h = self.model._enc_out
            if h is None or not h.requires_grad:
                raise CvaeError("overlap_exchange: the model did not take the fused path that exposes its encoder output")
            ga = torch.autograd.grad(res[0], params_a + [h], grad_outputs=ops.cached_one(res[0]), retain_graph=True, allow_unused=True)
            for p, g in zip(params_a, ga[:-1]):
                p.grad = g
            gh = ga[-1]
            self.out = tuple(r.detach() for r in res)
            self.red_a.pack()
        self.g1b = torch.cuda.CUDAGraph()
        with _capture(self.g1b, pool=self.g1.pool(), stream=cap):
            gb = torch.autograd.grad(h, params_b, grad_outputs=gh, allow_unused=True)
            for p, g in zip(params_b, gb):
                p.grad = g
            self.red_b.pack()
        self.model._enc_out = None
        del h, gh, ga, gb, res
        self.g2 = torch.cuda.CUDAGraph()
        with _capture(self.g2, pool=self.g1.pool(), stream=cap):
            self.red_a.bind_views()
            self.red_b.bind_views()
            self.opt.step()

    def _reduce_eager(self):
        if self.reducer is not None:
            self.reducer()

    def __call__(self, x=None, m=None, t=None):
        if x is not None:
            self.x.copy_(x, non_blocking=True)
        if m is not None:
            self.m.copy_(m, non_blocking=True)
        if t is not None:
            self.t.copy_(t, non_blocking=True)
        self.g1.replay()
        if self.g1b is not None:
            wa = self.red_a.all_reduce_async()
            self.g1b.replay()
            wb = self.red_b.all_reduce_async()
            for w in (wa, wb):
                if w is not None:
                    w.wait()
            self.g2.replay()
        elif self.g2 is not None:
            self.reducer.all_reduce()
            self.g2.replay()
        return self.out


class GraphedCallable:

    def __init__(self, fn, warmup=3):
        side = torch.cuda.Stream()
        side.wait_stream(torch.cuda.current_stream())
        with torch.cuda.stream(side):
            for _ in range(warmup):
                fn()
        torch.cuda.current_stream().wait_stream(side)
        torch.cuda.synchronize()
        self.graph = torch.cuda.CUDAGraph()
        with _capture(self.graph):
            self.out = fn()

    def __call__(self):
        self.graph.replay()
        return self.out
```

### causal_vae_amd/ops.py

```python
import ctypes as C_
import math

import torch

from . import _lib as L
from ._lib import lib, check, ptr, stream


_SIDE = {}
FORK_BACKWARD = False
FORK_MAX_POSITIONS = 0
DEFER_JOIN = False
_PENDING = {}


class _Fork:

    def __init__(self, device, positions=None):
        self.main = torch.cuda.current_stream(device)
        key = (device.index if device.index is not None else torch.cuda.current_device())
        self.key = key
        if key not in _SIDE:
            _SIDE[key] = torch.cuda.Stream(device=device)
        on = FORK_BACKWARD and (FORK_MAX_POSITIONS <= 0 or positions is None or positions <= FORK_MAX_POSITIONS)
# ... 1302 lines not shown
        return buf[0], buf[1], buf[2], buf[3]

    @staticmethod
    def backward(ctx, g_loss, g_recon, g_m, g_kld):
        src, x, m_hat, m, mu, logvar, t1 = ctx.saved_tensors
        if g_recon is not None or g_m is not None or g_kld is not None:
            raise L.CvaeError("ElboUp2x back-propagates the total loss only; for a single term use loss_function on the model's recon_x")
        if g_loss is None:
            return None, None, None, None, None, None, None, None
        B, d, h, w, Cc, D, H, W = ElboUp2x.dims(src, x)
        dsrc, d_mhat, dmu, dlv = torch.empty_like(src), torch.empty_like(m_hat), torch.empty_like(mu), torch.empty_like(mu)
        check(lib.cvae_elbo_up2x_bwd(ptr(t1), ptr(m_hat), ptr(m), ptr(mu), ptr(logvar), ctx.gamma, ptr(g_loss.contiguous()), ptr(dsrc),
                                     ptr(d_mhat), ptr(dmu), ptr(dlv), B, d, h, w, D, H, W, m.numel(), mu.numel(), L.dtype_code(src.dtype), stream()), "elbo_up2x_bwd")
        return dsrc, None, d_mhat, None, dmu, dlv, None, None


class WeightedSum(torch.autograd.Function):

    @staticmethod
    def forward(ctx, weights, *terms):
        import ctypes as C
        L.require_gpu(*terms)
        n = len(terms)
        if not 1 <= n <= 8 or len(weights) != n:
            raise L.CvaeError("WeightedSum: 1..8 terms, one weight each")
        ts = [t.float().contiguous() for t in terms]
        if any(t.numel() != 1 for t in ts):
            raise L.CvaeError("WeightedSum: scalar (0-dim) terms expected")
        out = torch.empty(n + 1, dtype=torch.float32, device=ts[0].device)
        check(lib.cvae_weighted_sum((C.c_void_p * n)(*[t.data_ptr() for t in ts]), (C.c_float * n)(*[float(w) for w in weights]), n, None, ptr(out), 0, stream()), "weighted_sum")
        ctx.weights = [float(w) for w in weights]
        ctx.shapes = [t.shape for t in terms]
        total, parts = out[0], out[1:]
        ctx.mark_non_differentiable(parts)
        ctx.set_materialize_grads(False)
        return total, parts

    @staticmethod
    def backward(ctx, g, _gparts):
        if g is None:
            return (None,) * (1 + len(ctx.weights))
        import ctypes as C
        n = len(ctx.weights)
        out = torch.empty(n, dtype=torch.float32, device=g.device)
        check(lib.cvae_weighted_sum(None, (C.c_float * n)(*ctx.weights), n, ptr(g.float().contiguous()), ptr(out), 1, stream()), "weighted_sum_bwd")
        return (None,) + tuple(out[i].view(ctx.shapes[i]) for i in range(n))


def weighted_sum(terms, weights, return_terms=False):
    total, parts = WeightedSum.apply(tuple(weights), *terms)
    return (total, parts) if return_terms else total


def sse(a, b):
    return _PairLoss.apply(a, b, "sse")


def bce_sum(p, x):
    return _PairLoss.apply(p, x, "bce")


class VesselRecon(torch.autograd.Function):

    @staticmethod
    def forward(ctx, r, x, sync=False, group=None):
        L.require_gpu(r, x)
        r, x = r.contiguous(), x.contiguous()
        sx = _scalar(r)
        out2 = torch.zeros(2, dtype=torch.float32, device=r.device)
        _t, wp, wb = _red_ws(r)
        check(lib.cvae_sum_fwd(ptr(x), ptr(sx), x.numel(), wp, wb, stream()), "sum_fwd")
        n_pos = x.numel()
        if sync and _group_size(group) > 1:
            _all_reduce_sum(sx, group)
            n_pos *= _group_size(group)
        check(lib.cvae_wmse_sparsity_fwd(ptr(r), ptr(x), ptr(sx), ptr(out2), r.numel(), n_pos, wp, wb, stream()), "wmse_sparsity_fwd")
        ctx.save_for_backward(r, x, sx)
        ctx.n_pos = n_pos
        return out2[0], out2[1]

    @staticmethod
    def backward(ctx, g_recon, g_sp):
        r, x, sx = ctx.saved_tensors
        dr = torch.empty_like(r)
        g_recon = g_recon.contiguous() if g_recon is not None else None
        g_sp = g_sp.contiguous() if g_sp is not None else None
        check(lib.cvae_wmse_sparsity_bwd(ptr(r), ptr(x), ptr(sx), ptr(g_recon), ptr(g_sp), ptr(dr), r.numel(), ctx.n_pos, stream()), "wmse_sparsity_bwd")
        return dr, None, None, None


class GaussNLL(torch.autograd.Function):

    @staticmethod
    def forward(ctx, m, mu, logvar):
        L.require_gpu(m, mu, logvar)
        m, mu, logvar = m.contiguous(), mu.contiguous(), logvar.contiguous()
        out = _scalar(m)
        _t, wp, wb = _red_ws(m)
        check(lib.cvae_gauss_nll_fwd(ptr(m), ptr(mu), ptr(logvar), ptr(out), m.numel(), wp, wb, stream()), "gauss_nll_fwd")
        ctx.save_for_backward(m, mu, logvar)
        return out

    @staticmethod
    def backward(ctx, g):
        m, mu, logvar = ctx.saved_tensors
        g = g.contiguous()
        dmu, dlv = torch.empty_like(mu), torch.empty_like(mu)
        check(lib.cvae_gauss_nll_bwd(ptr(m), ptr(mu), ptr(logvar), ptr(g), ptr(dmu), ptr(dlv), m.numel(), stream()), "gauss_nll_bwd")
        return None, dmu, dlv


class SoftmaxCE(torch.autograd.Function):

    @staticmethod
    def forward(ctx, logits, target):
        L.require_gpu(logits, target)
        logits, target = logits.contiguous(), target.contiguous()
        out = _scalar(logits)
        _t, wp, wb = _red_ws(logits)
        check(lib.cvae_softmax_ce_fwd(ptr(logits), ptr(target), ptr(out), logits.shape[0], logits.shape[1], wp, wb, stream()), "softmax_ce_fwd")
        ctx.save_for_backward(logits, target)
        return out

    @staticmethod
    def backward(ctx, g):
        logits, target = ctx.saved_tensors
        g = g.contiguous()
        dl = torch.empty_like(logits)
        check(lib.cvae_softmax_ce_bwd(ptr(logits), ptr(target), ptr(g), ptr(dl), logits.shape[0], logits.shape[1], stream()), "softmax_ce_bwd")
        return dl, None


class UniformKL(torch.autograd.Function):

    @staticmethod
    def forward(ctx, logits):
        L.require_gpu(logits)
        logits = logits.contiguous()
        out = _scalar(logits)
        _t, wp, wb = _red_ws(logits)
        check(lib.cvae_uniform_kl_fwd(ptr(logits), ptr(out), logits.shape[0], logits.shape[1], wp, wb, stream()), "uniform_kl_fwd")
        ctx.save_for_backward(logits)
        return out

    @staticmethod
    def backward(ctx, g):
        (logits,) = ctx.saved_tensors
        g = g.contiguous()
        dl = torch.empty_like(logits)
        check(lib.cvae_uniform_kl_bwd(ptr(logits), ptr(g), ptr(dl), logits.shape[0], logits.shape[1], stream()), "uniform_kl_bwd")
        return dl


class BioBottleneck(torch.autograd.Function):

    @staticmethod
    def supported(y_cl, out_size, training, widths=None):
        B, D, H, W, C = y_cl.shape
        OD, OH, OW = out_size
        ok = training and 2 <= B <= 16 and C % 64 == 0 and D % OD == 0 and H % OH == 0 and W % OW == 0
        if ok and widths is not None:
            dims = L.BottleneckDims(B, D, H, W, C, OD, OH, OW, *widths)
            ok = lib.cvae_bottleneck_sizes(C_.byref(dims), None, None, None, None, None) == 0
        return ok

    @staticmethod
    def forward(ctx, y_cl, m, t_onehot, eps, *rest):
        params, (rm, rv, nbt, momentum, bn_eps, out_size), sync = rest[:18], rest[18:24], (rest[24] if len(rest) > 24 else None)
        noise = rest[25] if len(rest) > 25 else None
        ctx.n_extra = len(rest) - 18
        L.require_gpu(y_cl, m, t_onehot, eps, *params)
        params = [p.contiguous() for p in params]
        W1, W2, Wmu, Wm0 = params[0], params[2], params[4], params[8]
        t_labels = None
        if t_onehot.dim() == 1 and not t_onehot.is_floating_point():
            t_labels = t_onehot.contiguous().long()
            t_onehot = torch.empty(t_labels.shape[0], Wm0.shape[1], dtype=torch.float32, device=y_cl.device)
        y_cl, m, t_onehot, eps = y_cl.contiguous(), m.contiguous().float(), t_onehot.contiguous().float(), eps.contiguous().float()
        B, D, H, W, C = y_cl.shape
        dims = L.BottleneckDims(B, D, H, W, C, *out_size, m.shape[1], t_onehot.shape[1], W1.shape[0], W2.shape[0], Wmu.shape[0], Wm0.shape[0])
        sizes = [C_.c_int64() for _ in range(5)]
        check(lib.cvae_bottleneck_sizes(C_.byref(dims), *[C_.byref(v) for v in sizes]), "bottleneck_sizes")
        K1, K4, n_fwd, n_dzm, n_dx = (v.value for v in sizes)
        if W1.shape[1] != K1 or params[16].shape != (C * out_size[0] * out_size[1] * out_size[2], K4):
            raise L.CvaeError(f"BioBottleneck: enc_fc.0 expects {W1.shape[1]} inputs, the pooled features + m + t give {K1}")
        dev, f32 = y_cl.device, torch.float32
        new = lambda *shape: torch.empty(*shape, dtype=f32, device=dev)
        xcat, partial, dzm_acc = new(B, K1), new(n_fwd), new(n_dzm)
        N1, N2, Z, HM, DM = dims.N1, dims.N2, dims.Z, dims.HM, dims.m_dim
        saved = dict(h1=new(B, N1), h2=new(B, N2), mu=new(B, Z), logvar=new(B, Z), xhat=new(B, HM), invstd=new(HM), a1n=new(B, HM), a2=new(B, HM),
                     m_hat=new(B, DM), zm=new(B, K4))
        dec_cl = torch.empty(B, *out_size, C, dtype=y_cl.dtype, device=dev)
        pstruct = L.BottleneckPtrs18(*[ptr(p) for p in params])
        sstruct = L.BottleneckSaved(*[ptr(saved[k]) for k in L.BOTTLENECK_SAVED])
        rank_stats, ranks = None, 0
        if sync is not None:
            rank_stats = sync[1].contiguous()
            ranks = rank_stats.shape[0]
            if tuple(rank_stats.shape) != (ranks, 2, HM) or rank_stats.dtype != f32:
                raise L.CvaeError(f"BioBottleneck: sync rank_stats must be float32 [ranks, 2, {HM}], got {tuple(rank_stats.shape)}")
        nstruct = None
        if noise is not None:
            if noise[2].dtype != torch.int32 or noise[2].device != dev:
                raise L.CvaeError("BioBottleneck: the noise call counter must be an int32 tensor on the activations' device")
            nstruct = C_.byref(L.BottleneckNoise(int(noise[0]), int(noise[1]), ptr(noise[2])))
        check(lib.cvae_bottleneck_fwd(C_.byref(dims), C_.byref(pstruct), ptr(y_cl), ptr(m), ptr(t_onehot), ptr(t_labels), ptr(eps), ptr(rm), ptr(rv), ptr(nbt), float(momentum),
                                      float(bn_eps), 1, ptr(xcat), ptr(partial), ptr(dzm_acc), C_.byref(sstruct), ptr(dec_cl), L.dtype_code(y_cl.dtype), ptr(rank_stats), ranks,
                                      nstruct, stream()), "bottleneck_fwd")
        ctx.dims, ctx.scratch = dims, n_dx
        ctx.sync = None if sync is None else (sync[0], ranks)
        ctx.save_for_backward(y_cl, t_onehot, eps, xcat, *params, *[saved[k] for k in L.BOTTLENECK_SAVED], dzm_acc)
        ctx.mark_non_differentiable(*[t for t in (rm, rv, nbt) if t is not None])
        return saved["mu"], saved["logvar"], saved["m_hat"], dec_cl

    @staticmethod
    def backward(ctx, g_mu, g_logvar, g_mhat, g_dec):
        y_cl, t_onehot, eps, xcat = ctx.saved_tensors[:4]
        params, saved, dzm_part = ctx.saved_tensors[4:22], ctx.saved_tensors[22:-1], ctx.saved_tensors[-1]
        dims, n_dx = ctx.dims, ctx.scratch
        dev, f32 = y_cl.device, torch.float32
        if g_dec is None:
            g_dec = torch.zeros(dims.M, dims.OD, dims.OH, dims.OW, dims.C, dtype=y_cl.dtype, device=dev)
        fix = lambda g: None if g is None else g.contiguous().float()
        g_mu, g_logvar, g_mhat, g_dec = fix(g_mu), fix(g_logvar), fix(g_mhat), g_dec.contiguous()
        grads = [torch.empty_like(p) for p in params]
        g1, dx_part = (torch.empty(n, dtype=f32, device=dev) for n in (dims.M * (dims.N1 + dims.N2), n_dx))
        dy_cl = torch.empty_like(y_cl)
        pstruct = L.BottleneckPtrs18(*[ptr(p) for p in params])
        gstruct = L.BottleneckPtrs18(*[ptr(g) for g in grads])
        sstruct = L.BottleneckSaved(*[ptr(t) for t in saved])
        bn_dy = bn_sums = None
        if ctx.sync is not None:
            bn_dy, bn_sums = torch.empty(dims.M, dims.HM, dtype=f32, device=dev), torch.empty(2, dims.HM, dtype=f32, device=dev)
        check(lib.cvae_bottleneck_bwd(C_.byref(dims), C_.byref(pstruct), C_.byref(gstruct), C_.byref(sstruct), ptr(g_dec), ptr(g_mu), ptr(g_logvar), ptr(g_mhat),
                                      ptr(t_onehot), ptr(eps), ptr(xcat), ptr(y_cl), 1, ptr(dzm_part), ptr(g1), ptr(dx_part), ptr(dy_cl),
                                      L.dtype_code(y_cl.dtype), ptr(bn_dy), ptr(bn_sums), stream()), "bottleneck_bwd")
        if ctx.sync is not None:
            group, ranks = ctx.sync
            _all_reduce_sum(bn_sums, group)
            check(lib.cvae_bottleneck_bn_bwd_finish(C_.byref(dims), C_.byref(pstruct), C_.byref(gstruct), C_.byref(sstruct), ptr(t_onehot), ptr(bn_dy), ptr(bn_sums), ranks,
                                                    stream()), "bottleneck_bn_bwd_finish")
        return (dy_cl, None, None, None, *grads, *([None] * ctx.n_extra))


def bottleneck_bn_rank_stats(Wm0, bm0, t, group=None):
    import torch.distributed as dist
    L.require_gpu(Wm0, bm0, t)
    Wm0, bm0 = Wm0.contiguous(), bm0.contiguous()
    HM, T = Wm0.shape
    labels = t.contiguous().long() if (t.dim() == 1 and not t.is_floating_point()) else None
    onehot = None if labels is not None else t.contiguous().float()
    B = t.shape[0]
    local = torch.empty(2, HM, dtype=torch.float32, device=Wm0.device)
    check(lib.cvae_bottleneck_bn_local_stats(ptr(Wm0), ptr(bm0), ptr(onehot), ptr(labels), ptr(local), B, T, HM, stream()), "bottleneck_bn_local_stats")
    world = _group_size(group)
    if world == 1:
        return local.unsqueeze(0)
    parts = [torch.empty_like(local) for _ in range(world)]
    dist.all_gather(parts, local, group=group)
    return torch.stack(parts)


class BatchNorm2dAct(torch.autograd.Function):

    @staticmethod
    def forward(ctx, x, weight, bias, running_mean, running_var, momentum, eps, training, act):
        L.require_gpu(x, weight, bias)
        x = x.contiguous()
        Cc = x.shape[-1]
        P = x.numel() // Cc
        y = torch.empty_like(x)
        if training:
            mean, rstd = _empty((Cc,), torch.float32, x), _empty((Cc,), torch.float32, x)
        else:
            mean, rstd = running_mean.float().clone(), torch.rsqrt(running_var.float() + eps)
        _t, wp, wb = _scratch(lib.cvae_bn2d_workspace_bytes(P, Cc) if training else 0, x)
        check(lib.cvae_bn2d_fwd(ptr(x), ptr(weight), ptr(bias), ptr(y), ptr(mean), ptr(rstd), ptr(running_mean) if training else None,
                                ptr(running_var) if training else None, P, Cc, float(momentum), float(eps), 1 if training else 0, L.act_code(act),
                                L.dtype_code(x.dtype), wp, wb, stream()), "bn2d_fwd")
        ctx.save_for_backward(x, y, weight, mean, rstd)
        ctx.cfg = (training, act)
        return y

    @staticmethod
    def backward(ctx, g):
        x, y, weight, mean, rstd = ctx.saved_tensors
        training, act = ctx.cfg
        if not training:
            raise L.CvaeError("BatchNorm2d in eval mode is forward-only here (the reference consumers run it under no_grad)")
        Cc = x.shape[-1]
        P = x.numel() // Cc
        g = g.contiguous()
        dx = torch.empty_like(x)
        dw, db = _empty((Cc,), torch.float32, x), _empty((Cc,), torch.float32, x)
        _t, wp, wb = _scratch(lib.cvae_bn2d_workspace_bytes(P, Cc), x)
        check(lib.cvae_bn2d_bwd(ptr(x), ptr(g), ptr(y), ptr(weight), ptr(mean), ptr(rstd), ptr(dx), ptr(dw), ptr(db), P, Cc, L.act_code(act),
                                L.dtype_code(x.dtype), wp, wb, stream()), "bn2d_bwd")
        return dx, dw, db, None, None, None, None, None, None


class Clamp(torch.autograd.Function):

    @staticmethod
    def forward(ctx, x, lo, hi):
        L.require_gpu(x)
        x = x.contiguous().float()
        y = torch.empty_like(x)
        check(lib.cvae_clamp_fwd(ptr(x), ptr(y), float(lo), float(hi), x.numel(), stream()), "clamp_fwd")
        ctx.save_for_backward(x)
        ctx.lim = (float(lo), float(hi))
        return y

    @staticmethod
    def backward(ctx, g):
        (x,) = ctx.saved_tensors
        g = g.contiguous()
        dx = torch.empty_like(x)
        check(lib.cvae_clamp_bwd(ptr(x), ptr(g), ptr(dx), ctx.lim[0], ctx.lim[1], x.numel(), stream()), "clamp_bwd")
        return dx, None, None


class Conv3ToK4(torch.autograd.Function):

    @staticmethod
    def forward(ctx, w3):
        L.require_gpu(w3)
        w3 = w3.contiguous()
        Cout, Cin = w3.shape[0], w3.shape[1]
        if tuple(w3.shape[2:]) != (3, 3):
            raise L.CvaeError("Conv3ToK4: a [Cout, Cin, 3, 3] weight expected")
        k4 = torch.empty(Cin, Cout, 4, 4, dtype=torch.float32, device=w3.device)
        check(lib.cvae_conv3_to_k4(ptr(w3), ptr(k4), Cout, Cin, stream()), "conv3_to_k4")
        ctx.shape = (Cout, Cin)
        return k4

    @staticmethod
    def backward(ctx, g):
        Cout, Cin = ctx.shape
        g = g.contiguous()
        dw3 = torch.empty(Cout, Cin, 3, 3, dtype=torch.float32, device=g.device)
        check(lib.cvae_k4_to_conv3_grad(ptr(g), ptr(dw3), Cout, Cin, stream()), "k4_to_conv3_grad")
        return dw3


FOLD_CONV_K4, FOLD_UPCONV_K3, FOLD_CONV_K3S2 = 0, 1, 3
FOLD_CONVT_K3S2, FOLD_CONV_K3S1, FOLD_CONVT_K3S2_SUBPIXEL = 4, 5, 6
FOLD_CONV_K3S1_GRAD, FOLD_CONVT_K3S2_SUBPIXEL_GRAD = 7, 8
_FOLD_GRAD = (FOLD_CONV_K3S1_GRAD, FOLD_CONVT_K3S2_SUBPIXEL_GRAD)
_FOLD_CONVT = (FOLD_CONVT_K3S2, FOLD_CONVT_K3S2_SUBPIXEL, FOLD_CONVT_K3S2_SUBPIXEL_GRAD)
_FOLD_GEMM = (FOLD_CONV_K3S1, FOLD_CONVT_K3S2_SUBPIXEL) + _FOLD_GRAD


def _forward_only(what, *tensors):
    if torch.is_grad_enabled() and any(t is not None and t.requires_grad for t in tensors):
        raise L.CvaeError(f"{what} is forward-only (eval-mode inference): call it under torch.no_grad()")


def fold_bn_conv(entries):
    import ctypes as C
    k = len(entries)
    if not 1 <= k <= 16:
        raise L.CvaeError(f"fold_bn_conv: 1 to 16 layers per launch, got {k}")
    for w, kind, bias, bn in entries:
        L.require_gpu(w, bias)
        _forward_only("fold_bn_conv", w, bias, *((bn.weight, bn.bias) if bn is not None else ()))
        if bn is not None and (bn.running_mean is None or bn.weight is None):
            raise L.CvaeError("fold_bn_conv: the BatchNorm2d needs running statistics and an affine weight (eval mode, track_running_stats, affine)")
    sizes = []
    for w, kind, _b, _bn in entries:
        if (kind not in (FOLD_CONV_K4, FOLD_UPCONV_K3, FOLD_CONV_K3S2) + _FOLD_CONVT + _FOLD_GEMM or w.dim() != 4
                or tuple(w.shape[2:]) != ((4, 4) if kind == FOLD_CONV_K4 else (3, 3))):
            raise L.CvaeError(f"fold_bn_conv: kind {kind} does not match a weight of shape {tuple(w.shape)}")
        cout = w.shape[1] if kind in _FOLD_CONVT else w.shape[0]
        if kind in _FOLD_GEMM:
            cin, taps, rows = (w.shape[0], 4, 4 * cout) if kind in _FOLD_CONVT else (w.shape[1], 9, cout)
            nbwd = 0 if kind not in _FOLD_GRAD else (32 * 256 if kind in _FOLD_CONVT else cin * ((9 * cout + 63) // 64 * 64))
            sizes.append((rows * ((taps * cin + 63) // 64 * 64), cout, nbwd))
        else:
            sizes.append((w.shape[0] * w.shape[1] * 16, cout, 0))
    pad = lambda n: (n + 3) // 4 * 4
    buf = torch.empty(sum(pad(a + g) + pad(b) for a, b, g in sizes), dtype=torch.float32, device=entries[0][0].device)
    outs, off = [], 0
    for (w, kind, _b, _bn), (nw, nb, ng) in zip(entries, sizes):
        shape = tuple(w.shape[:2]) + (4, 4) if kind != FOLD_UPCONV_K3 else (w.shape[1], w.shape[0], 4, 4)
        if kind in _FOLD_GEMM:
            shape = (4 * nb if kind in _FOLD_CONVT else nb, -1)
        wo = buf[off:off + nw].view(shape)
        wg = buf[off + nw:off + nw + ng].view((32 if kind in _FOLD_CONVT else w.shape[1], -1)) if ng else None
        off += pad(nw + ng)
        bo = buf[off:off + nb]
        off += pad(nb)
        outs.append((wo, bo, wg) if ng else (wo, bo))
    ws = [w.contiguous() for w, _k, _b, _bn in entries]
    vp = lambda v: (C.c_void_p * k)(*v)
# ... 667 lines not shown
```

### causal_vae_amd/optim.py

```python
import torch

from . import _lib as L
from ._lib import lib, check, ptr, stream


class FusedAdam(torch.optim.Optimizer):

    def __init__(self, params, lr=1e-3, betas=(0.9, 0.999), eps=1e-8, device_step=False):
        super().__init__(params, dict(lr=lr, betas=betas, eps=eps))
        self.device_step = device_step
        self._step_dev = None
        self._early, self._early_hooks, self._side = [], [], None
        self._early_left, self._early_ran, self._counted = 0, False, False

    def overlap_backward(self, early_params):
        for h in self._early_hooks:
            h.remove()
        self._early_hooks, self._early = [], [p for p in early_params if p.requires_grad]
        if not self._early:
            return
        if len(self.param_groups) != 1:
            raise L.CvaeError("FusedAdam.overlap_backward: one parameter group expected")
        self._early_ids = {id(p) for p in self._early}
        self._early_left, self._early_ran = len(self._early), False
        for p in self._early:
            self._early_hooks.append(p.register_post_accumulate_grad_hook(self._early_hook))

    def _early_hook(self, p):
        self._early_left -= 1
        if self._early_left == 0:
            from . import ops
            ops.flush_pending_wgrads()
            main = torch.cuda.current_stream()
            if self._side is None:
                self._side = torch.cuda.Stream()
            with torch.no_grad():
                self._count_step(self._early[0].device)
                self._side.wait_stream(main)
                with torch.cuda.stream(self._side):
                    self._update(self.param_groups[0], self._early, None)
            self._early_ran = True

    def zero_grad(self, set_to_none=True):
        self._early_left, self._early_ran = len(self._early), False
        return super().zero_grad(set_to_none=set_to_none)

    def claim_step_counter(self, device):
        if not self.device_step:
            return None
        if self._step_dev is None:
            self._step_dev = torch.zeros((), dtype=torch.int32, device=device)
        self._counted = True
        return self._step_dev

    def _count_step(self, device):
        if self.device_step and not self._counted:
            if self._step_dev is None:
                self._step_dev = torch.zeros((), dtype=torch.int32, device=device)
            check(lib.cvae_counter_add(ptr(self._step_dev), 1, stream()), "counter_add")
            self._counted = True

    def _update(self, group, ps, grad_scale):
        import ctypes as C
        b1, b2 = group["betas"]
        L.require_gpu(*ps)
        t = None
        gs = []
        for p in ps:
            if p.dtype != torch.float32 or not p.is_contiguous():
                raise L.CvaeError("FusedAdam: contiguous float32 parameters expected")
            st = self.state[p]
            if not st:
                st["step"] = 0
                st["exp_avg"] = torch.zeros_like(p)
                st["exp_avg_sq"] = torch.zeros_like(p)
            st["step"] += 1
            if t is None:
                t = st["step"]
            elif t != st["step"]:
                raise L.CvaeError("FusedAdam: parameters of one group must share a step count")
            gs.append(p.grad if p.grad.is_contiguous() else p.grad.contiguous())
        n = len(ps)
        arr = lambda vals: (C.c_void_p * n)(*vals)
        sizes = (C.c_int64 * n)(*[p.numel() for p in ps])
        step_ptr = ptr(self._step_dev) if self.device_step else None
        check(lib.cvae_adam_multi(arr([p.data_ptr() for p in ps]), arr([g.data_ptr() for g in gs]),
                                  arr([self.state[p]["exp_avg"].data_ptr() for p in ps]),
                                  arr([self.state[p]["exp_avg_sq"].data_ptr() for p in ps]), sizes, n, group["lr"], b1, b2,
                                  group["eps"], 1.0 - b1 ** t, 1.0 - b2 ** t, step_ptr, ptr(grad_scale), stream()), "adam_multi")

    def _sync_step_from_device(self):
        if self.device_step and self._step_dev is not None:
            t = int(self._step_dev.item())
            for st in self.state.values():
                if "step" in st:
                    st["step"] = t

    def state_dict(self):
        self._sync_step_from_device()
        return super().state_dict()

    def load_state_dict(self, state_dict):
        old = {p: (st.get("exp_avg"), st.get("exp_avg_sq")) for p, st in self.state.items()}
        super().load_state_dict(state_dict)
        for p, st in self.state.items():
            for key, prev in zip(("exp_avg", "exp_avg_sq"), old.get(p, (None, None))):
                new = st.get(key)
                if prev is not None and new is not None and new is not prev and prev.shape == new.shape and prev.device == new.device:
                    prev.copy_(new)
                    st[key] = prev
        steps = {int(st["step"]) for st in self.state.values() if "step" in st}
        if len(steps) > 1:
            raise L.CvaeError("FusedAdam.load_state_dict: parameters carry different step counts")
        if self.device_step and steps:
            dev = next(iter(self.state)).device
            t = steps.pop()
            if self._step_dev is not None and self._step_dev.device == dev:
                self._step_dev.fill_(t)
            else:
                self._step_dev = torch.full((), t, dtype=torch.int32, device=dev)
        self._counted = False

    @torch.no_grad()
    def step(self, closure=None, grad_scale=None):
        loss = None
        if closure is not None:
            with torch.enable_grad():
                loss = closure()
        from . import ops
        ops.join_side_streams()
        early_done = self._early_ran
        if early_done and grad_scale is not None:
            raise L.CvaeError("FusedAdam: grad_scale cannot be combined with overlap_backward (part of the update has already run)")
        for group in self.param_groups:
            ps = [p for p in group["params"] if p.grad is not None and not (early_done and id(p) in self._early_ids)]
            if ps:
                self._count_step(ps[0].device)
                self._update(group, ps, grad_scale)
        if early_done:
            torch.cuda.current_stream().wait_stream(self._side)
        self._counted, self._early_ran, self._early_left = False, False, len(self._early)
        return loss


@torch.no_grad()
def clip_grad_norm_(parameters, max_norm, scale_grads=True):
    import ctypes as C
    from . import ops
    ops.join_side_streams()
    params = [p for p in parameters if p.grad is not None]
    if not params:
        return None, None
    dev = params[0].device
    sq = torch.zeros((), dtype=torch.float32, device=dev)
    coef = torch.empty((), dtype=torch.float32, device=dev)
    nws = int(lib.cvae_reduce_workspace_bytes())
    ws = torch.empty(nws // 4, dtype=torch.float32, device=dev)
    gs = []
    for p in params:
        if not p.grad.is_contiguous():
            p.grad = p.grad.contiguous()
        if p.grad.dtype != torch.float32:
            raise L.CvaeError("clip_grad_norm_: float32 gradients expected")
        gs.append(p.grad)
    n = len(gs)
    check(lib.cvae_sqnorm_multi((C.c_void_p * n)(*[g.data_ptr() for g in gs]), (C.c_int64 * n)(*[g.numel() for g in gs]), n, ptr(sq), ptr(ws), nws, stream()), "sqnorm_multi")
    check(lib.cvae_clip_coef(ptr(sq), ptr(coef), float(max_norm), stream()), "clip_coef")
    if scale_grads:
        for g in gs:
            check(lib.cvae_scale(ptr(g), g.numel(), ptr(coef), stream()), "scale")
    return sq, coef
```

### include/cvae_hip.h

```cpp
#ifndef CVAE_HIP_H
#define CVAE_HIP_H
#include <stddef.h>
#include <stdint.h>

#ifdef __cplusplus
extern "C" {
#endif

#define CVAE_OK             0
#define CVAE_E_BADSHAPE    (-1)
#define CVAE_E_DTYPE       (-2)
#define CVAE_E_UNSUPPORTED (-3)
#define CVAE_E_WORKSPACE   (-4)
#define CVAE_E_LAUNCH      (-5)
#define CVAE_E_NULLPTR     (-6)

#define CVAE_F32  0
#define CVAE_BF16 1
#define CVAE_FP8  2

#define CVAE_ACT_NONE    0
#define CVAE_ACT_RELU    1
#define CVAE_ACT_SIGMOID 2
#define CVAE_ACT_LEAKY02 3
// ... 131 lines not shown
int cvae_conv_s1_bwd_data(const void* g, const void* w, const void* resid, const void* gate, void* dx, int64_t B, int64_t H, int64_t W, int64_t C, int form,
                          int dtype, int gate_act, void* stream);
int cvae_conv_s1_c1_bwd_data(const float* g, const float* w, const void* gate, void* dx, int64_t B, int64_t H, int64_t W, int64_t Cin, int dtype, int gate_act,
                             void* stream);
size_t cvae_latent_to_grid_bwd_workspace_bytes(int64_t B, int64_t K, int64_t P, int64_t C);
int cvae_latent_to_grid_bwd(const void* g, const float* W, float* dz, int64_t B, int64_t K, int64_t P, int64_t C, int dtype, void* workspace, size_t workspace_bytes,
                            void* stream);
size_t cvae_conv_s1_wgrad_workspace_bytes(int64_t B, int64_t H, int64_t W, int64_t C, int form);
int cvae_conv_s1_wgrad(const void* x, const void* g, float* dW, float* dbias, int64_t B, int64_t H, int64_t W, int64_t C, int form, int dtype, void* workspace,
                       size_t workspace_bytes, void* stream);
size_t cvae_conv_s1_c1_wgrad_workspace_bytes(int64_t B, int64_t H, int64_t W);
int cvae_conv_s1_c1_wgrad(const void* x, const float* g, float* dW, float* dbias, int64_t B, int64_t H, int64_t W, int64_t Cin, int dtype, void* workspace,
                          size_t workspace_bytes, void* stream);
int cvae_latent_to_grid_wgrad(const void* g, const float* z, float* dW, float* dbias, int64_t B, int64_t K, int64_t P, int64_t C, int dtype, void* stream);

#define CVAE_HEADS_MAX_PANELS 3
#define CVAE_HEADS_MAX_LAYERS 3
#define CVAE_HEADS_MAX_WIDTH  512
typedef struct { const float* ptr; int64_t width, stride; } cvae_heads_panel;
typedef struct {
    const float *W, *b, *W2, *b2;
    int64_t out, out_first;
    const float *bn_weight, *bn_bias, *bn_mean, *bn_var;
    float bn_eps;
    int leaky;
    float slope;
} cvae_heads_layer;
int cvae_mlp_heads_fwd(const cvae_heads_panel* panels, int n_panels, const cvae_heads_layer* layers, int n_layers, int64_t split,
                       const float* clamp0, const float* clamp1, const float* eps, int64_t eps_stride, float* out0, int64_t out0_stride,
                       float* out1, int64_t out1_stride, float* z, int64_t z_stride, int64_t B, void* stream);

typedef struct { float *running_mean, *running_var; int64_t* num_batches_tracked; float momentum; } cvae_heads_bn_train;
typedef struct { float *dW, *db, *dW2, *db2, *dgamma, *dbeta; } cvae_heads_layer_grad;
size_t cvae_mlp_heads_train_workspace_bytes(const cvae_heads_panel* panels, int n_panels, const cvae_heads_layer* layers, int n_layers, int64_t B);
size_t cvae_mlp_heads_bwd_workspace_bytes(const cvae_heads_panel* panels, int n_panels, const cvae_heads_layer* layers, int n_layers, int64_t B);
int cvae_mlp_heads_train_fwd(const cvae_heads_panel* panels, int n_panels, const cvae_heads_layer* layers, int n_layers, const cvae_heads_bn_train* bn,
                             int64_t split, const float* clamp0, const float* clamp1, const float* eps, int64_t eps_stride, float* out0,
                             int64_t out0_stride, float* out1, int64_t out1_stride, float* z, int64_t z_stride, int64_t B, void* saved,
                             size_t saved_bytes, void* stream);
int cvae_mlp_heads_bwd(const cvae_heads_panel* panels, int n_panels, float* const* panel_grads, const int64_t* panel_grad_strides,
                       const cvae_heads_layer* layers, int n_layers, const cvae_heads_layer_grad* grads, int64_t split, const float* clamp0,
                       const float* clamp1, const float* eps, int64_t eps_stride, const float* g0, int64_t g0_stride, const float* g1,
                       int64_t g1_stride, const float* gz, int64_t gz_stride, int64_t B, const void* saved, size_t saved_bytes, void* workspace,
                       size_t workspace_bytes, void* stream);

typedef struct { int64_t M, D, H, W, C, OD, OH, OW, m_dim, t_dim, N1, N2, Z, HM; } cvae_bottleneck_dims;
typedef struct {
    const float *W1, *b1, *W2, *b2, *Wmu, *bmu, *Wlv, *blv, *Wm0, *bm0, *gamma, *beta, *Wm3, *bm3, *Wm5, *bm5, *Wd, *bd;
} cvae_bottleneck_params;
typedef struct {
    float *dW1, *db1, *dW2, *db2, *dWmu, *dbmu, *dWlv, *dblv, *dWm0, *dbm0, *dgamma, *dbeta, *dWm3, *dbm3, *dWm5, *dbm5, *dWd, *dbd;
} cvae_bottleneck_grads;
typedef struct {
    float *h1, *h2, *mu, *logvar, *xhat, *invstd, *a1n, *a2, *m_hat, *zm;
} cvae_bottleneck_saved;
int cvae_bottleneck_sizes(const cvae_bottleneck_dims* dims, int64_t* K1, int64_t* K4, int64_t* fwd_partial_floats, int64_t* dzm_partial_floats,
                          int64_t* dx_partial_floats);
typedef struct { uint64_t seed, subsequence; int* call_counter; } cvae_bottleneck_noise;
int cvae_bottleneck_fwd(const cvae_bottleneck_dims* dims, const cvae_bottleneck_params* params, const void* y_cl, const float* m, float* t_onehot,
                        const int64_t* t_labels, float* eps, float* running_mean, float* running_var, long long* num_batches_tracked, float momentum,
                        float bn_eps, int bn_training, float* xcat, float* fwd_partial, float* dzm_acc, const cvae_bottleneck_saved* saved, void* dec_cl, int dtype,
                        const float* bn_rank_stats, int bn_ranks, const cvae_bottleneck_noise* noise, void* stream);
int cvae_bottleneck_bwd(const cvae_bottleneck_dims* dims, const cvae_bottleneck_params* params, const cvae_bottleneck_grads* grads,
                        const cvae_bottleneck_saved* saved, const void* g_dec_cl, const float* g_mu, const float* g_logvar, const float* g_mhat,
                        const float* t_onehot, const float* eps, const float* xcat, const void* y_cl, int relu_mask, float* dzm_partial, float* g1,
                        float* dx_partial, void* dy_cl, int dtype, float* bn_dy, float* bn_local_sums, void* stream);

int cvae_bottleneck_bn_local_stats(const float* Wm0, const float* bm0, const float* t_onehot, const int64_t* t_labels, float* local_stats, int64_t M, int64_t t_dim,
                                   int64_t HM, void* stream);
int cvae_bottleneck_bn_bwd_finish(const cvae_bottleneck_dims* dims, const cvae_bottleneck_params* params, const cvae_bottleneck_grads* grads,
                                  const cvae_bottleneck_saved* saved, const float* t_onehot, const float* bn_dy, const float* bn_sums, int bn_ranks, void* stream);

size_t cvae_conv_wgrad_workspace_bytes(int64_t Cs, int64_t Cl, int nd);
int cvae_conv_wgrad(const void* S, const void* L, float* dW, float* dbias, int dbias_side, void* workspace, size_t workspace_bytes,
                    int64_t B, int64_t sd, int64_t sh, int64_t sw, int64_t Cs,
                    int64_t ld, int64_t lh, int64_t lw, int64_t Cl, int nd, int dtype, void* stream);
int cvae_conv_wgrad_multi(int count, const void* const* S, const void* const* L, float* const* dW, float* const* dbias, const int* dbias_side,
                          void* const* workspace, const size_t* workspace_bytes, const int64_t* dims, int nd, int dtype, void* stream);
size_t cvae_channel_sum_workspace_bytes(int64_t P, int64_t C, int dtype);
int cvae_channel_sum(const void* x, float* out, int64_t P, int64_t C, int dtype, void* workspace, size_t workspace_bytes, void* stream);
int cvae_act_fwd(const void* x, void* y, int64_t n, int act, int dtype, void* stream);
int cvae_act_bwd(const void* dy, const void* y, void* dx, int64_t n, int act, int dtype, void* stream);

int cvae_adaptive_avgpool_fwd(const void* x, float* out, int64_t B, int64_t D, int64_t H, int64_t W, int64_t C,
                              int64_t OD, int64_t OH, int64_t OW, int64_t out_stride, int dtype, void* stream);
int cvae_adaptive_avgpool_bwd(const float* dout, const void* relu_mask_x, void* dx, int64_t B, int64_t D, int64_t H, int64_t W, int64_t C,
                              int64_t OD, int64_t OH, int64_t OW, int64_t dout_stride, int dtype, void* stream);
int cvae_upsample_linear_fwd(const void* src, float* dst, int64_t B, int64_t d, int64_t h, int64_t w,
                             int64_t D, int64_t H, int64_t W, int64_t C, int dtype, void* stream);
int cvae_upsample_linear_bwd(const float* ddst, void* dsrc, int64_t B, int64_t d, int64_t h, int64_t w,
                             int64_t D, int64_t H, int64_t W, int64_t C, int dtype, void* stream);

size_t cvae_linear_workspace_bytes(int64_t M, int64_t K, int64_t N, int op);
int cvae_linear_fwd(const float* x, const float* W, const float* b, float* y, int64_t M, int64_t K, int64_t N,
                    int64_t x_stride, int64_t y_stride, int act, int bf16_math, void* workspace, size_t workspace_bytes, void* stream);
int cvae_linear_bwd_data(const float* dy, const float* W, float* dx, int64_t M, int64_t K, int64_t N, int64_t dy_stride, int64_t dx_stride,
                         const float* y_act, int act, const float* x_in, int64_t x_stride, int in_act, int bf16_math,
                         void* workspace, size_t workspace_bytes, void* stream);
int cvae_linear_bwd_weight(const float* dy, const float* x, float* dW, float* db, int64_t M, int64_t K, int64_t N,
                           int64_t dy_stride, int64_t x_stride, const float* y_act, int act, int bf16_math, void* workspace, size_t workspace_bytes,
                           void* stream);

int cvae_bn1d_train_fwd(const float* x, const float* w, const float* b, float* y, float* save_mean, float* save_rstd,
                        float* running_mean, float* running_var, int64_t B, int64_t F, float momentum, float eps, void* stream);
int cvae_bn1d_train_bwd(const float* dy, const float* x, const float* w, const float* save_mean, const float* save_rstd,
                        float* dx, float* dw, float* db, int64_t B, int64_t F, void* stream);
int cvae_bn1d_eval_fwd(const float* x, const float* w, const float* b, const float* running_mean, const float* running_var,
                       float* y, int64_t B, int64_t F, float eps, void* stream);
int cvae_bn1d_stats(const float* x, const float* mean_sum, float inv_n, float* out, int64_t B, int64_t F, void* stream);
int cvae_bn1d_apply_stats(const float* x, const float* w, const float* b, const float* mean_sum, const float* sqdev_sum, float inv_n, float* y,
                          float* save_mean, float* save_rstd, float* running_mean, float* running_var, int64_t B, int64_t F, float momentum,
                          float eps, void* stream);
int cvae_bn1d_bwd_sums(const float* dy, const float* x, const float* save_mean, const float* save_rstd, float* sums, int64_t B, int64_t F, void* stream);
int cvae_bn1d_bwd_apply(const float* dy, const float* x, const float* w, const float* save_mean, const float* save_rstd, const float* sums, float inv_n,
                        float* dx, int64_t B, int64_t F, void* stream);

size_t cvae_reduce_workspace_bytes(void);
int cvae_philox_normal(float* out, int64_t n, uint64_t seed, uint64_t offset, uint64_t subsequence, const int* call_counter, void* stream);
int cvae_philox_normal_advance(float* out, int64_t n, uint64_t seed, uint64_t offset, uint64_t subsequence, int* call_counter, void* stream);
int cvae_reparam_kld_fwd(const float* mu, const float* logvar, const float* eps, float* z, float* kld, int64_t n, void* workspace, size_t workspace_bytes, void* stream);
int cvae_reparam_kld_bwd(const float* dz, const float* gkld, float gk_scale, const float* mu, const float* logvar, const float* eps,
                         float* dmu, float* dlogvar, int64_t n, void* stream);
int cvae_latent_head_fwd(const float* h, const float* eps1, const float* eps2, float* z1, float* z2, float* kld, int64_t B, int64_t Z, void* stream);
int cvae_latent_head_bwd(const float* dz1, const float* dz2, const float* gkld, const float* h, const float* eps1, const float* eps2, float* dh,
                         int64_t B, int64_t Z, void* stream);
int cvae_sse_fwd(const float* a, const float* b, float* out, int64_t n, void* workspace, size_t workspace_bytes, void* stream);
int cvae_sse_bwd(const float* a, const float* b, const float* gout, float scale, float* da, int64_t n, void* stream);
int cvae_combine3(float* out4, float wb, float wc, void* stream);
int cvae_bce_fwd(const float* p, const float* x, float* out, int64_t n, void* workspace, size_t workspace_bytes, void* stream);
int cvae_bce_bwd(const float* p, const float* x, const float* gout, float* dp, int64_t n, void* stream);
int cvae_sum_fwd(const float* x, float* out, int64_t n, void* workspace, size_t workspace_bytes, void* stream);
int cvae_wmse_sparsity_fwd(const float* r, const float* x, const float* sum_x, float* out2, int64_t n, int64_t n_pos, void* workspace, size_t workspace_bytes, void* stream);
int cvae_wmse_sparsity_bwd(const float* r, const float* x, const float* sum_x, const float* g_recon, const float* g_sparsity,
                           float* dr, int64_t n, int64_t n_pos, void* stream);
int cvae_gauss_nll_fwd(const float* m, const float* mu, const float* logvar, float* out, int64_t n, void* workspace, size_t workspace_bytes, void* stream);
int cvae_gauss_nll_bwd(const float* m, const float* mu, const float* logvar, const float* gout, float* dmu, float* dlogvar, int64_t n, void* stream);
int cvae_softmax_ce_fwd(const float* logits, const int64_t* target, float* out, int64_t B, int64_t C, void* workspace, size_t workspace_bytes, void* stream);
int cvae_softmax_ce_bwd(const float* logits, const int64_t* target, const float* gout, float* dlogits, int64_t B, int64_t C, void* stream);
int cvae_uniform_kl_fwd(const float* logits, float* out, int64_t B, int64_t C, void* workspace, size_t workspace_bytes, void* stream);
int cvae_uniform_kl_bwd(const float* logits, const float* gout, float* dlogits, int64_t B, int64_t C, void* stream);

int cvae_small_dense_supported(int64_t M, int64_t K, int64_t N);
size_t cvae_small_dense_workspace_bytes(int64_t M, int64_t K, int64_t N);
int cvae_small_dense_fwd(const float* x, const float* W, const float* b, float* y, int64_t M, int64_t K, int64_t N, int64_t x_stride, int64_t y_stride, int act, void* stream);
int cvae_small_dense_bwd_data(const float* dy, const float* W, float* dx, const float* y_act, int act, const float* x_in, int in_act, int64_t M, int64_t K, int64_t N,
                              int64_t dy_stride, int64_t dx_stride, int64_t y_stride, int64_t x_stride, void* stream);
int cvae_small_dense_bwd_weight(const float* dy, const float* x, float* dW, float* db, const float* y_act, int act, int64_t M, int64_t K, int64_t N, int64_t dy_stride,
                                int64_t x_stride, int64_t y_stride, void* workspace, size_t workspace_bytes, void* stream);

int cvae_adam_step(float* p, const float* g, float* m, float* v, int64_t n, float lr, float beta1, float beta2, float eps,
                   float bc1, float bc2, const float* grad_scale, void* stream);
int cvae_adam_multi(float* const* p, const float* const* g, float* const* m, float* const* v, const int64_t* n, int count,
                    float lr, float beta1, float beta2, float eps, float bc1, float bc2, const int* step_dev,
                    const float* grad_scale, void* stream);
int cvae_multi_copy(const float* const* src, float* const* dst, const int64_t* n, int count, void* stream);
int cvae_counter_add(int* counter, int delta, void* stream);
int cvae_sqnorm(const float* g, float* out, int64_t n, void* workspace, size_t workspace_bytes, void* stream);
int cvae_weighted_sum(const float* const* terms, const float* weights, int count, const float* g, float* out, int backward, void* stream);
int cvae_sqnorm_multi(const float* const* g, const int64_t* n, int count, float* out, void* workspace, size_t workspace_bytes, void* stream);
int cvae_scale(float* g, int64_t n, const float* scale, void* stream);
int cvae_clip_coef(const float* sqnorm, float* scale, float max_norm, void* stream);

#ifdef __cplusplus
}
#endif
#endif
```

Measured before the change: 5206 samples/s.

## Fuse rank-M W1 weight gradient into Adam instead of materializing dW1

The bottleneck backward no longer writes the dense dW1 for the large first FC layer. The optimizer instead receives the low-rank factors (g1 and xcat, rank equal to the batch size) and recomputes each gradient element inside the multi-tensor Adam kernel. This removes one full write and one full read of a dW1-sized buffer per step, at the cost of an M-term dot product per element inside Adam. Summation order is kept bitwise-matched through the fused/unfused FMA helpers. Gradient clipping and grad_scale cannot be combined with the factored gradient.

```diff
diff --git a/causal_vae_amd/_lib.py b/causal_vae_amd/_lib.py
--- a/causal_vae_amd/_lib.py
+++ b/causal_vae_amd/_lib.py
@@ -97,7 +97,7 @@
     "cvae_uniform_kl_fwd": [_p, _p, _i64, _i64, _p, _sz, _p],
     "cvae_uniform_kl_bwd": [_p, _p, _p, _i64, _i64, _p],
     "cvae_adam_step": [_p, _p, _p, _p, _i64, _f, _f, _f, _f, _f, _f, _p, _p],
-    "cvae_adam_multi": [_p, _p, _p, _p, _p, _i, _f, _f, _f, _f, _f, _f, _p, _p, _p],
+    "cvae_adam_multi": [_p, _p, _p, _p, _p, _i, _f, _f, _f, _f, _f, _f, _p, _p, _p, _p, _p, _p],
     "cvae_multi_copy": [_p, _p, _p, _i, _p],
     "cvae_counter_add": [_p, _i, _p],
     "cvae_sqnorm": [_p, _p, _i64, _p, _sz, _p],
diff --git a/causal_vae_amd/csrc/bottleneck.hip b/causal_vae_amd/csrc/bottleneck.hip
--- a/causal_vae_amd/csrc/bottleneck.hip
+++ b/causal_vae_amd/csrc/bottleneck.hip
@@ -806,7 +806,9 @@
 struct __attribute__((packed, aligned(4))) F2U { float x, y; };
 template <int MT> struct SkinnyBwdCols { static constexpr int value = 4; using vec = F4U; };
 template <> struct SkinnyBwdCols<16> { static constexpr int value = 2; using vec = F2U; };
-template <int MT>
+static_assert(SkinnyBwdCols<4>::value == lowrank_vec_cols(4) && SkinnyBwdCols<8>::value == lowrank_vec_cols(8) && SkinnyBwdCols<16>::value == lowrank_vec_cols(16),
+              "lowrank_vec_cols (common.h) tells the Adam rebuild which columns of dW1 took the tail loop");
+template <int MT, bool WRITE_DW>
 __global__ __launch_bounds__(256) void skinny_bwd_colwise_kernel(const float* __restrict__ g, const float* __restrict__ x, const float* __restrict__ Wt,
                                                                  float* __restrict__ dW, float* __restrict__ dxp, int M, int K, int N, int nslice, int F, int S,
                                                                  int NS, TailDims d, TailParams tp, TailGrads tg, TailSaved sv, MechBwdArgs mb) {
@@ -846,9 +848,12 @@
                 for (int m = 0; m < MT; ++m) {
                     const float gv = gs[m][j];
 #pragma unroll
-                    for (int c = 0; c < CPT; ++c) { dwf[c] += gv * xv[m][c]; acc[m][c] += gv * wf[c]; }
+                    for (int c = 0; c < CPT; ++c) {
+                        if constexpr (WRITE_DW) dwf[c] = lowrank_term(dwf[c], gv, xv[m][c]);
+                        acc[m][c] += gv * wf[c];
+                    }
                 }
-                st_stream<typename SkinnyBwdCols<MT>::vec>(dW + (size_t)(nb + j) * K + k0, dw);
+                if constexpr (WRITE_DW) st_stream<typename SkinnyBwdCols<MT>::vec>(dW + (size_t)(nb + j) * K + k0, dw);
             }
         } else if (nk > 0) {
             for (int j = 0; j < cnt; ++j)
@@ -856,8 +861,11 @@
                     const float w = Wt[(size_t)(nb + j) * K + k0 + c];
                     float dw = 0.f;
 #pragma unroll
-                    for (int m = 0; m < MT; ++m) { dw += gs[m][j] * xv[m][c]; acc[m][c] += gs[m][j] * w; }
-                    dW[(size_t)(nb + j) * K + k0 + c] = dw;
+                    for (int m = 0; m < MT; ++m) {
+                        if constexpr (WRITE_DW) dw = lowrank_term_tail(dw, gs[m][j], xv[m][c], tail_term_fused(MT, m));
+                        acc[m][c] += gs[m][j] * w;
+                    }
+                    if constexpr (WRITE_DW) dW[(size_t)(nb + j) * K + k0 + c] = dw;
                 }
         }
     }
@@ -948,7 +956,8 @@
 int bwd_lds_ready(const TailDims& d) {
     const int rc = with_mt(d.M, [&](auto mt) {
         constexpr int MT = decltype(mt)::value;
-        return cvae_allow_lds<skinny_bwd_colwise_kernel<MT>>(mech_bwd_lds(d), bwd_colwise_static(MT));
+        const int r = cvae_allow_lds<skinny_bwd_colwise_kernel<MT, true>>(mech_bwd_lds(d), bwd_colwise_static(MT));
+        return r == CVAE_OK ? cvae_allow_lds<skinny_bwd_colwise_kernel<MT, false>>(mech_bwd_lds(d), bwd_colwise_static(MT)) : r;
     });
     return rc == CVAE_OK ? cvae_allow_lds<fc2_bwd_kernel>(fc2_bwd_lds(d)) : rc;
 }
@@ -1095,9 +1104,11 @@
     CVAE_CHECK_LAUNCH();
     const MechBwdArgs mb{dzm_partial, g_mhat, t_onehot, bn_dy, bn_local_sums};
     with_mt(M, [&](auto mt) {
+      with_bool(gr->dW1 != nullptr, [&](auto write_dw) {
         constexpr int MT = decltype(mt)::value, COLS = 256 * SkinnyBwdCols<MT>::value;
-        hipLaunchKernelGGL(skinny_bwd_colwise_kernel<MT>, dim3((unsigned)((K1 + COLS - 1) / COLS), (unsigned)(NS + 1)), dim3(256), mech_bwd_lds(d), st, (const float*)g1, xcat,
+        hipLaunchKernelGGL((skinny_bwd_colwise_kernel<MT, decltype(write_dw)::value>), dim3((unsigned)((K1 + COLS - 1) / COLS), (unsigned)(NS + 1)), dim3(256), mech_bwd_lds(d), st, (const float*)g1, xcat,
                            w->W1, gr->dW1, dx_partial, M, K1, (int)q->N1, ((int)q->N1 + NS - 1) / NS, F, S, NS, d, p, g, s, mb);
+      });
     });
     CVAE_CHECK_LAUNCH();
     with_dtype(dtype, [&](auto tv) {
diff --git a/causal_vae_amd/csrc/common.h b/causal_vae_amd/csrc/common.h
--- a/causal_vae_amd/csrc/common.h
+++ b/causal_vae_amd/csrc/common.h
@@ -192,6 +192,16 @@
 template <typename F> auto with_dtype(int dtype, F&& f) { return dtype == CVAE_BF16 ? f(bf16{}) : f(float{}); }
 template <typename F> auto with_epi(int act, F&& f) { return CVAE_EPI_OF(act) == 0 ? f(Int<0>{}) : (CVAE_EPI_OF(act) == 1 ? f(Int<1>{}) : f(Int<2>{})); }
 template <typename F> auto with_bool(bool b, F&& f) { return b ? f(std::true_type{}) : f(std::false_type{}); }
+__host__ __device__ constexpr int lowrank_vec_cols(int M) { return M <= 8 ? 4 : 2; }
+__host__ __device__ constexpr int lowrank_tail_begin(int M, int K) { return K - K % lowrank_vec_cols(M); }
+__device__ __forceinline__ float lowrank_term(float acc, float a, float b) { return __builtin_fmaf(a, b, acc); }
+__host__ __device__ constexpr bool tail_term_fused(int M, int m) { return M > 8 && m < 4; }
+__device__ __forceinline__ float lowrank_term_tail(float acc, float a, float b, bool fused) {
+#pragma clang fp contract(off)
+    if (fused) return __builtin_fmaf(a, b, acc);
+    const float p = a * b;
+    return acc + p;
+}
 __device__ __forceinline__ float act_grad_from_out(float y, int act) {
     switch (act) {
         case CVAE_ACT_RELU: return y > 0.f ? 1.f : 0.f;
diff --git a/causal_vae_amd/csrc/losses.hip b/causal_vae_amd/csrc/losses.hip
--- a/causal_vae_amd/csrc/losses.hip
+++ b/causal_vae_amd/csrc/losses.hip
@@ -601,6 +601,15 @@
     v = b2 * v + (1.f - b2) * g * g;
     p -= step * (m / (sqrtf(v) * rbc2 + eps));
 }
+template <bool FUSED>
+__device__ __forceinline__ void adam1_multi(float& p, float g, float& m, float& v, float b1, float b2, float eps, float step, float rbc2) {
+#pragma clang fp contract(off)
+    const float bm = b1 * m, bv = b2 * v, t = (1.f - b2) * g;
+    if (FUSED) { m = __builtin_fmaf(1.f - b1, g, bm); v = __builtin_fmaf(g, t, bv); }
+    else { const float gm = (1.f - b1) * g, tg = t * g; m = bm + gm; v = bv + tg; }
+    const float q = m / __builtin_fmaf(sqrtf(v), rbc2, eps);
+    p = __builtin_fmaf(-step, q, p);
+}
 __global__ void adam_kernel(float* __restrict__ p, const float* __restrict__ g, float* __restrict__ m, float* __restrict__ v, int64_t n,
                             float lr, float b1, float b2, float eps, float bc1, float bc2, const float* __restrict__ gscale) {
     const float gs = gscale ? *gscale : 1.f;
@@ -633,6 +642,7 @@
     return CVAE_OK;
 }
 #define ADAM_MAX_TENSORS 64
+#define ADAM_MAX_RANK 16
 #define ADAM_SPAN 4096
 #define ADAM_MULTI_SPAN 1024
 struct AdamTable {
@@ -641,9 +651,74 @@
     float* m[ADAM_MAX_TENSORS];
     float* v[ADAM_MAX_TENSORS];
     long long n[ADAM_MAX_TENSORS];
+    const float* xb[ADAM_MAX_TENSORS];
+    int fk[ADAM_MAX_TENSORS];
+    unsigned char fm[ADAM_MAX_TENSORS];
     int blk_start[ADAM_MAX_TENSORS + 1];
     int count;
 };
+static_assert(sizeof(AdamTable) + 64 <= 4096, "the table and the scalars travel as kernel arguments");
+__device__ __forceinline__ float adam_factored_grad1(const float* __restrict__ ga, const float* __restrict__ xb, int M, int N, int K, int kt, long long n, int k) {
+    float a = 0.f;
+    if (k < kt) for (int mm = 0; mm < M; ++mm) a = lowrank_term(a, ga[(size_t)mm * N + n], xb[(size_t)mm * K + k]);
+    else for (int mm = 0; mm < M; ++mm) a = lowrank_term_tail(a, ga[(size_t)mm * N + n], xb[(size_t)mm * K + k], tail_term_fused(M, mm));
+    return a;
+}
+typedef float adam_f4u __attribute__((ext_vector_type(4), aligned(4)));
+__device__ __forceinline__ float4 adam_factored_grad4(const float* __restrict__ ga, const float* __restrict__ xb, int M, int N, int K, int kt, long long n, int k) {
+    float a[4] = {0.f, 0.f, 0.f, 0.f};
+    if (k + 4 <= kt) {
+#pragma unroll 4
+        for (int mm = 0; mm < M; ++mm) {
+            const float gv = ga[(size_t)mm * N + n];
+            const adam_f4u x = *(const adam_f4u*)(xb + (size_t)mm * K + k);
+            a[0] = lowrank_term(a[0], gv, x.x); a[1] = lowrank_term(a[1], gv, x.y); a[2] = lowrank_term(a[2], gv, x.z); a[3] = lowrank_term(a[3], gv, x.w);
+        }
+    } else {
+#pragma unroll
+        for (int c = 0; c < 4; ++c) {
+            a[c] = adam_factored_grad1(ga, xb, M, N, K, kt, n, k);
+            if (++k == K) { k = 0; ++n; }
+        }
+    }
+    return make_float4(a[0], a[1], a[2], a[3]);
+}
+template <int SPAN, bool NT>
+__device__ __forceinline__ void adam_factored_span(float* __restrict__ p, const float* __restrict__ ga, const float* __restrict__ xb, float* __restrict__ m,
+                                                   float* __restrict__ v, long long n, int fM, int fK, long long base, long long end, float gs, float b1,
+                                                   float b2, float eps, float step, float rbc2) {
+    const int fN = (int)(n / fK), fkt = lowrank_tail_begin(fM, fK);
+    const long long fn0 = base / fK;
+    const int fk0 = (int)(base - fn0 * fK);
+    const bool vec = ((((uintptr_t)p) | ((uintptr_t)m) | ((uintptr_t)v)) & 15) == 0;
+    if (vec && end - base == SPAN) {
+#pragma unroll
+        for (int k = 0; k < SPAN / (256 * 4); ++k) {
+            const long long i = base / 4 + k * 256 + threadIdx.x;
+            const int kk = fk0 + 4 * (k * 256 + (int)threadIdx.x), dn = kk / fK;
+            const float4 G = adam_factored_grad4(ga, xb, fM, fN, fK, fkt, fn0 + dn, kk - dn * fK);
+            float4 P, M, V;
+            typedef float f4v __attribute__((ext_vector_type(4)));
+            if (NT) {
+                f4v a = __builtin_nontemporal_load((f4v*)p + i), c = __builtin_nontemporal_load((f4v*)m + i), d = __builtin_nontemporal_load((f4v*)v + i);
+                P = make_float4(a.x, a.y, a.z, a.w); M = make_float4(c.x, c.y, c.z, c.w); V = make_float4(d.x, d.y, d.z, d.w);
+            } else { P = ((float4*)p)[i]; M = ((float4*)m)[i]; V = ((float4*)v)[i]; }
+            adam1_multi<true>(P.x, G.x * gs, M.x, V.x, b1, b2, eps, step, rbc2);
+            adam1_multi<true>(P.y, G.y * gs, M.y, V.y, b1, b2, eps, step, rbc2);
+            adam1_multi<true>(P.z, G.z * gs, M.z, V.z, b1, b2, eps, step, rbc2);
+            adam1_multi<true>(P.w, G.w * gs, M.w, V.w, b1, b2, eps, step, rbc2);
+            if (NT) {
+                f4v a = {P.x, P.y, P.z, P.w}, c = {M.x, M.y, M.z, M.w}, d = {V.x, V.y, V.z, V.w};
+                __builtin_nontemporal_store(a, (f4v*)p + i); __builtin_nontemporal_store(c, (f4v*)m + i); __builtin_nontemporal_store(d, (f4v*)v + i);
+            } else { ((float4*)p)[i] = P; ((float4*)m)[i] = M; ((float4*)v)[i] = V; }
+        }
+    } else {
+        for (long long i = base + threadIdx.x; i < end; i += 256) {
+            const long long nn = i / fK;
+            adam1_multi<false>(p[i], adam_factored_grad1(ga, xb, fM, fN, fK, fkt, nn, (int)(i - nn * fK)) * gs, m[i], v[i], b1, b2, eps, step, rbc2);
+        }
+    }
+}
 template <int SPAN, bool NT = false>
 __global__ __launch_bounds__(256) void adam_multi_kernel(AdamTable tb, float lr, float b1, float b2, float eps, float bc1, float bc2,
                                                          const int* __restrict__ step_dev, const float* __restrict__ gscale) {
@@ -656,6 +731,7 @@
     const long long n = tb.n[ti];
     const long long base = (long long)((int)blockIdx.x - tb.blk_start[ti]) * SPAN;
     const long long end = min(n, base + SPAN);
+    if (tb.xb[ti]) { adam_factored_span<SPAN, NT>(p, g, tb.xb[ti], m, v, n, tb.fm[ti], tb.fk[ti], base, end, gs, b1, b2, eps, step, rbc2); return; }
     const bool vec = ((((uintptr_t)p) | ((uintptr_t)g) | ((uintptr_t)m) | ((uintptr_t)v)) & 15) == 0;
     if (vec && end - base == SPAN) {
 #pragma unroll
@@ -668,10 +744,10 @@
                 f4v c = __builtin_nontemporal_load((f4v*)m + i), d = __builtin_nontemporal_load((f4v*)v + i);
                 P = make_float4(a.x, a.y, a.z, a.w); G = make_float4(b.x, b.y, b.z, b.w); M = make_float4(c.x, c.y, c.z, c.w); V = make_float4(d.x, d.y, d.z, d.w);
             } else { P = ((float4*)p)[i]; G = ((const float4*)g)[i]; M = ((float4*)m)[i]; V = ((float4*)v)[i]; }
-            adam1(P.x, G.x * gs, M.x, V.x, b1, b2, eps, step, rbc2);
-            adam1(P.y, G.y * gs, M.y, V.y, b1, b2, eps, step, rbc2);
-            adam1(P.z, G.z * gs, M.z, V.z, b1, b2, eps, step, rbc2);
-            adam1(P.w, G.w * gs, M.w, V.w, b1, b2, eps, step, rbc2);
+            adam1_multi<true>(P.x, G.x * gs, M.x, V.x, b1, b2, eps, step, rbc2);
+            adam1_multi<true>(P.y, G.y * gs, M.y, V.y, b1, b2, eps, step, rbc2);
+            adam1_multi<true>(P.z, G.z * gs, M.z, V.z, b1, b2, eps, step, rbc2);
+            adam1_multi<true>(P.w, G.w * gs, M.w, V.w, b1, b2, eps, step, rbc2);
             if (NT) {
                 typedef float f4v __attribute__((ext_vector_type(4)));
                 f4v a = {P.x, P.y, P.z, P.w}, c = {M.x, M.y, M.z, M.w}, d = {V.x, V.y, V.z, V.w};
@@ -680,14 +756,16 @@
             else { ((float4*)p)[i] = P; ((float4*)m)[i] = M; ((float4*)v)[i] = V; }
         }
     } else {
-        for (long long i = base + threadIdx.x; i < end; i += 256) adam1(p[i], g[i] * gs, m[i], v[i], b1, b2, eps, step, rbc2);
+        for (long long i = base + threadIdx.x; i < end; i += 256) adam1_multi<false>(p[i], g[i] * gs, m[i], v[i], b1, b2, eps, step, rbc2);
     }
 }
 extern "C" int cvae_adam_multi(float* const* p, const float* const* g, float* const* m, float* const* v, const int64_t* n, int count,
-                               float lr, float b1, float b2, float eps, float bc1, float bc2, const int* step_dev, const float* gscale, void* stream) {
+                               float lr, float b1, float b2, float eps, float bc1, float bc2, const int* step_dev, const float* gscale,
+                               const float* const* g_right, const int64_t* g_rank, const int64_t* g_cols, void* stream) {
     if (count < 0) return CVAE_E_BADSHAPE;
     if (count == 0) return CVAE_OK;
     if (!p || !g || !m || !v || !n) return CVAE_E_NULLPTR;
+    if (g_right && (!g_rank || !g_cols)) return CVAE_E_NULLPTR;
     if (!step_dev && (bc1 <= 0.f || bc2 <= 0.f)) return CVAE_E_BADSHAPE;
     const int span = ADAM_MULTI_SPAN;
     for (int c0 = 0; c0 < count; c0 += ADAM_MAX_TENSORS) {
@@ -700,6 +778,12 @@
             if (ni == 0) continue;
             if (!p[c0 + i] || !g[c0 + i] || !m[c0 + i] || !v[c0 + i]) return CVAE_E_NULLPTR;
             tb.p[used] = p[c0 + i]; tb.g[used] = g[c0 + i]; tb.m[used] = m[c0 + i]; tb.v[used] = v[c0 + i]; tb.n[used] = ni;
+            tb.xb[used] = g_right ? g_right[c0 + i] : nullptr; tb.fk[used] = 0; tb.fm[used] = 0;
+            if (tb.xb[used]) {
+                const int64_t M = g_rank[c0 + i], K = g_cols[c0 + i];
+                if (M < 1 || M > ADAM_MAX_RANK || K < 1 || K > INT32_MAX - span || ni % K || ni / K > INT32_MAX) return CVAE_E_BADSHAPE;
+                tb.fk[used] = (int)K; tb.fm[used] = (unsigned char)M;
+            }
             tb.blk_start[used] = blocks;
             blocks += (int)((ni + span - 1) / span);
             ++used;
diff --git a/causal_vae_amd/graph.py b/causal_vae_amd/graph.py
--- a/causal_vae_amd/graph.py
+++ b/causal_vae_amd/graph.py
@@ -30,6 +30,7 @@
         _check_sync_bn_capturable(model)
         self.x, self.m, self.t = (b.clone() for b in batch)
         self.loss_fn = loss_fn
+        self._factored = (not overlap_exchange and (reducer is None or not reducer.active()) and not getattr(optimizer, "_early", None))
         side = torch.cuda.Stream()
         side.wait_stream(torch.cuda.current_stream())
         with torch.cuda.stream(side):
@@ -63,7 +64,8 @@
             res = self.model.forward_elbo(self.x, self.m, self.t, bump=bump)
         else:
             res = self.loss_fn(self.model(self.x, self.m, self.t), self.x, self.m)
-        ops.backward_from(res[0])
+        with ops.factored_wgrads(self.opt if self._factored else None):
+            ops.backward_from(res[0])
         return tuple(r.detach() for r in res)
 
     def _capture_split(self):
diff --git a/causal_vae_amd/ops.py b/causal_vae_amd/ops.py
--- a/causal_vae_amd/ops.py
+++ b/causal_vae_amd/ops.py
@@ -1478,6 +1478,23 @@
         return dl
 
 
+FACTORED_WGRAD = True
+_FACTORED_SINK = [None]
+
+
+class factored_wgrads:
+
+    def __init__(self, sink):
+        self.sink = sink if FACTORED_WGRAD else None
+
+    def __enter__(self):
+        self.prev, _FACTORED_SINK[0] = _FACTORED_SINK[0], self.sink
+
+    def __exit__(self, *exc):
+        _FACTORED_SINK[0] = self.prev
+        return False
+
+
 class BioBottleneck(torch.autograd.Function):
 
     @staticmethod
@@ -1495,6 +1512,7 @@
         params, (rm, rv, nbt, momentum, bn_eps, out_size), sync = rest[:18], rest[18:24], (rest[24] if len(rest) > 24 else None)
         noise = rest[25] if len(rest) > 25 else None
         ctx.n_extra = len(rest) - 18
+        ctx.w1_param = rest[0]
         L.require_gpu(y_cl, m, t_onehot, eps, *params)
         params = [p.contiguous() for p in params]
         W1, W2, Wmu, Wm0 = params[0], params[2], params[4], params[8]
@@ -1549,7 +1567,10 @@
             g_dec = torch.zeros(dims.M, dims.OD, dims.OH, dims.OW, dims.C, dtype=y_cl.dtype, device=dev)
         fix = lambda g: None if g is None else g.contiguous().float()
         g_mu, g_logvar, g_mhat, g_dec = fix(g_mu), fix(g_logvar), fix(g_mhat), g_dec.contiguous()
-        grads = [torch.empty_like(p) for p in params]
+        sink = _FACTORED_SINK[0]
+        factored = (sink is not None and ctx.sync is None and ctx.needs_input_grad[4] and params[0].dtype == f32
+                    and params[0].data_ptr() == ctx.w1_param.data_ptr())
+        grads = [None if (factored and i == 0) else torch.empty_like(p) for i, p in enumerate(params)]
         g1, dx_part = (torch.empty(n, dtype=f32, device=dev) for n in (dims.M * (dims.N1 + dims.N2), n_dx))
         dy_cl = torch.empty_like(y_cl)
         pstruct = L.BottleneckPtrs18(*[ptr(p) for p in params])
@@ -1566,6 +1587,8 @@
             _all_reduce_sum(bn_sums, group)
             check(lib.cvae_bottleneck_bn_bwd_finish(C_.byref(dims), C_.byref(pstruct), C_.byref(gstruct), C_.byref(sstruct), ptr(t_onehot), ptr(bn_dy), ptr(bn_sums), ranks,
                                                     stream()), "bottleneck_bn_bwd_finish")
+        if factored:
+            sink.add_factored_grad(ctx.w1_param, g1[:dims.M * dims.N1].view(dims.M, dims.N1), xcat)
         return (dy_cl, None, None, None, *grads, *([None] * ctx.n_extra))
 
 
diff --git a/causal_vae_amd/optim.py b/causal_vae_amd/optim.py
--- a/causal_vae_amd/optim.py
+++ b/causal_vae_amd/optim.py
@@ -12,6 +12,7 @@
         self._step_dev = None
         self._early, self._early_hooks, self._side = [], [], None
         self._early_left, self._early_ran, self._counted = 0, False, False
+        self._factored, self._factored_spent = {}, set()
 
     def overlap_backward(self, early_params):
         for h in self._early_hooks:
@@ -41,7 +42,29 @@
                     self._update(self.param_groups[0], self._early, None)
             self._early_ran = True
 
+    def add_factored_grad(self, param, left, right):
+        own = None
+        for group in self.param_groups:
+            for p in group["params"]:
+                if p is param or (p.data_ptr() == param.data_ptr() and p.shape == param.shape):
+                    own = p
+        if own is None:
+            raise L.CvaeError("FusedAdam.add_factored_grad: the parameter does not belong to this optimizer")
+        if id(own) in self._factored or own.grad is not None:
+            raise L.CvaeError("FusedAdam.add_factored_grad: the parameter already holds a gradient for this step (factored gradients do not accumulate)")
+        if self._early and id(own) in self._early_ids:
+            raise L.CvaeError("FusedAdam.add_factored_grad: the parameter is updated early (overlap_backward)")
+        M = left.shape[0]
+        if (own.dim() != 2 or left.dim() != 2 or right.dim() != 2 or not 1 <= M <= 16 or right.shape[0] != M or (left.shape[1], right.shape[1]) != tuple(own.shape)
+                or left.dtype != torch.float32 or right.dtype != torch.float32 or not left.is_contiguous() or not right.is_contiguous()):
+            raise L.CvaeError(f"FusedAdam.add_factored_grad: factors {tuple(left.shape)} x {tuple(right.shape)} do not make a {tuple(own.shape)} gradient")
+        L.require_gpu(left, right)
+        self._factored[id(own)] = (own, left, right)
+        self._factored_spent.discard(id(own))
+
     def zero_grad(self, set_to_none=True):
+        self._factored.clear()
+        self._factored_spent.clear()
         self._early_left, self._early_ran = len(self._early), False
         return super().zero_grad(set_to_none=set_to_none)
 
@@ -79,15 +102,25 @@
                 t = st["step"]
             elif t != st["step"]:
                 raise L.CvaeError("FusedAdam: parameters of one group must share a step count")
-            gs.append(p.grad if p.grad.is_contiguous() else p.grad.contiguous())
+            fg = self._factored.get(id(p))
+            if fg is not None:
+                gs.append(fg[1])
+            else:
+                gs.append(p.grad if p.grad.is_contiguous() else p.grad.contiguous())
         n = len(ps)
         arr = lambda vals: (C.c_void_p * n)(*vals)
         sizes = (C.c_int64 * n)(*[p.numel() for p in ps])
         step_ptr = ptr(self._step_dev) if self.device_step else None
+        right = rank = cols = None
+        fgs = [self._factored.get(id(p)) for p in ps]
+        if any(fg is not None for fg in fgs):
+            right = arr([None if fg is None else fg[2].data_ptr() for fg in fgs])
+            rank = (C.c_int64 * n)(*[0 if fg is None else fg[1].shape[0] for fg in fgs])
+            cols = (C.c_int64 * n)(*[0 if fg is None else fg[2].shape[1] for fg in fgs])
         check(lib.cvae_adam_multi(arr([p.data_ptr() for p in ps]), arr([g.data_ptr() for g in gs]),
                                   arr([self.state[p]["exp_avg"].data_ptr() for p in ps]),
                                   arr([self.state[p]["exp_avg_sq"].data_ptr() for p in ps]), sizes, n, group["lr"], b1, b2,
-                                  group["eps"], 1.0 - b1 ** t, 1.0 - b2 ** t, step_ptr, ptr(grad_scale), stream()), "adam_multi")
+                                  group["eps"], 1.0 - b1 ** t, 1.0 - b2 ** t, step_ptr, ptr(grad_scale), right, rank, cols, stream()), "adam_multi")
 
     def _sync_step_from_device(self):
         if self.device_step and self._step_dev is not None:
@@ -132,11 +165,20 @@
         early_done = self._early_ran
         if early_done and grad_scale is not None:
             raise L.CvaeError("FusedAdam: grad_scale cannot be combined with overlap_backward (part of the update has already run)")
+        if self._factored and grad_scale is not None:
+            raise L.CvaeError("FusedAdam: grad_scale cannot be combined with a factored gradient (the clipping norm never saw it)")
         for group in self.param_groups:
-            ps = [p for p in group["params"] if p.grad is not None and not (early_done and id(p) in self._early_ids)]
+            for p in group["params"]:
+                if id(p) in self._factored and p.grad is not None:
+                    raise L.CvaeError("FusedAdam: a parameter holds both a factored and a dense gradient")
+                if id(p) in self._factored_spent and p.grad is None:
+                    raise L.CvaeError("FusedAdam: step() called again after a factored gradient was used up (its factors are gone: run backward first)")
+            ps = [p for p in group["params"] if (p.grad is not None or id(p) in self._factored) and not (early_done and id(p) in self._early_ids)]
             if ps:
                 self._count_step(ps[0].device)
                 self._update(group, ps, grad_scale)
+        self._factored_spent.update(self._factored)
+        self._factored.clear()
         if early_done:
             torch.cuda.current_stream().wait_stream(self._side)
         self._counted, self._early_ran, self._early_left = False, False, len(self._early)
diff --git a/include/cvae_hip.h b/include/cvae_hip.h
--- a/include/cvae_hip.h
+++ b/include/cvae_hip.h
@@ -307,7 +307,7 @@
                    float bc1, float bc2, const float* grad_scale, void* stream);
 int cvae_adam_multi(float* const* p, const float* const* g, float* const* m, float* const* v, const int64_t* n, int count,
                     float lr, float beta1, float beta2, float eps, float bc1, float bc2, const int* step_dev,
-                    const float* grad_scale, void* stream);
+                    const float* grad_scale, const float* const* g_right, const int64_t* g_rank, const int64_t* g_cols, void* stream);
 int cvae_multi_copy(const float* const* src, float* const* dst, const int64_t* n, int count, void* stream);
 int cvae_counter_add(int* counter, int delta, void* stream);
 int cvae_sqnorm(const float* g, float* out, int64_t n, void* workspace, size_t workspace_bytes, void* stream);
```

New measurement: 5212 samples/s (median of 2 runs). No clear change (+0.1%).
